# iKrishneel/fcn_object_detector

Measured on AMD Instinct MI355X. Metric: frames/sec forward 448x448 @1 GPU; train imgs/sec @1/2/4/8 GPUs, higher is better.
Workload: dtype f32; 1 GPU; configs[1]: single-GPU forward, DetectNet GoogLeNet conv stack + coverage/bbox heads (graph of models/deploy.prototxt), batch=1, 448x448, random-init weights; global_batch=1, parallelism=replicas x1, frames_in_flight=4

## Files before the change

### fcn_object_detector_amd/csrc/common.h

```cpp
#pragma once

#include <hip/hip_runtime.h>
#include <stdint.h>
#include <stdio.h>
#include <string.h>

#include "../../include/fcnhip.h"

namespace fcn {

char* err_buf();
int set_err(int code, const char* fmt, ...);

inline hipStream_t as_stream(fcn_stream_t s) { return reinterpret_cast<hipStream_t>(s); }

#define FCN_HIP(call)                                                                         \
    do {                                                                                      \
        hipError_t e__ = (call);                                                              \
        if (e__ != hipSuccess)                                                                \
            return ::fcn::set_err(-(int)e__, "%s failed: %s", #call, hipGetErrorString(e__)); \
    } while (0)

#define FCN_LAUNCH_CHECK(name)                                                                \
    do {                                                                                      \
        hipError_t e__ = hipGetLastError();                                                   \
        if (e__ != hipSuccess)                                                                \
            return ::fcn::set_err(-(int)e__, "launch %s failed: %s", name, hipGetErrorString(e__)); \
    } while (0)

#define FCN_REQUIRE(cond, code, ...)                         \
    do {                                                     \
        if (!(cond)) return ::fcn::set_err(code, __VA_ARGS__); \
    } while (0)

const float* zero_page_for_current_device(int* rc);

inline int cdiv(long long a, long long b) { return (int)((a + b - 1) / b); }

inline int stream_grid(long long work_items, int block) {
    long long g = (work_items + block - 1) / block;
    if (g < 1) g = 1;
    if (g > 65536) g = 8192;
    return (int)g;
}

}
```

### fcn_object_detector_amd/csrc/conv_fwd.hip

```cpp
#include <cstddef>
#include <algorithm>
#include <mutex>
#include <unordered_map>
#include <type_traits>

#include "common.h"
#include "conv_common.h"

using namespace fcn;

namespace fcn {

const float* zero_page_for_current_device(int* rc) {
    static std::mutex mu;
    static const float* pages[64] = {nullptr};
    int dev = 0;
    *rc = 0;
    if (hipGetDevice(&dev) != hipSuccess || dev < 0 || dev >= 64) {
        *rc = set_err(FCN_E_STATE, "conv: no current device");
        return nullptr;
    }
    std::lock_guard<std::mutex> lock(mu);
    if (!pages[dev]) {
        void* ptr = nullptr;
// ... 896 lines not shown
__global__ __launch_bounds__((Cfg<WTM, WTN, WAVES_M, WAVES_N, WAVES_K, BK, NBUF, PF>::NT)) void conv_fwd_group(const int nprob, const int te0, const int te1, const int te2,
                                                                                  const int te3, const int te4, const int te5, const int te6,
                                                                                  const int te7, const int pool_wgs, const int snake,
                                                                                  const std::conditional_t<TAIL, GroupArgsTail, GroupArgs> a_) {
    __shared__ __attribute__((aligned(16))) float smem[Cfg<WTM, WTN, WAVES_M, WAVES_N, WAVES_K, BK, NBUF, PF>::LDS_FLOATS + (TAIL ? kTailLdsFloats : 0)];
    const GroupArgs& a = group_of(a_);
    typedef unsigned u32x16 __attribute__((ext_vector_type(16)));
    typedef unsigned u32x8 __attribute__((ext_vector_type(8)));
    typedef const GroupArgs __attribute__((address_space(4))) * karg_ptr;
    static_assert(alignof(GroupArgsTail) == alignof(GroupArgs) && offsetof(GroupArgsTail, g) == 0, "the group leads its tail");
    constexpr size_t kArgsOffset = (11 * sizeof(int) + alignof(GroupArgs) - 1) / alignof(GroupArgs) * alignof(GroupArgs);
    karg_ptr ka = (karg_ptr)((const char __attribute__((address_space(4)))*)__builtin_amdgcn_kernarg_segment_ptr() + kArgsOffset);
    const int head[1 + kMaxGroup] = {nprob, te0, te1, te2, te3, te4, te5, te6, te7};
    static_assert(kMaxGroup == 8, "the tile prefix travels as eight scalar kernel arguments");
    const int pool_first = pool_wgs > 0 ? pool_wgs : 0;
    if ((int)blockIdx.x < pool_first || (pool_wgs < 0 && (int)blockIdx.x >= te7)) {
        const int w = pool_wgs < 0 ? (int)blockIdx.x - te7 : (int)blockIdx.x;
        if (w < a.pool[0].wg_end) pool_body<T, Cfg<WTM, WTN, WAVES_M, WAVES_N, WAVES_K, BK, NBUF, PF>::NT>(a.pool[0], w);
        else pool_body<T, Cfg<WTM, WTN, WAVES_M, WAVES_N, WAVES_K, BK, NBUF, PF>::NT>(a.pool[1], w - a.pool[0].wg_end);
        return;
    }
    int pos = blockIdx.x;
    if (snake > 0) {
        const int sh = snake & 255, rounds = snake >> 8;
        const int r = pos >> sh, j = pos & ((1 << sh) - 1);
        if (r > 0 && r < rounds - 1 && ((rounds - 1 - r) & 1)) pos = (r << sh) + ((1 << sh) - 1 - j);
    }
    int tile = pos - pool_first;
    if (snake == (int)0x80000000) {
        const int x = pos & 7, sl = pos >> 3, q = te7 >> 3, r = te7 & 7;
        tile = x * q + (x < r ? x : r) + sl;
    } else if (snake < 0) {
        tile += snake;
        tile += tile < 0 ? te7 : 0;
    }
    int pi = 0, begin = 0;
#pragma unroll
    for (int i = 0; i < kMaxGroup - 1; ++i) {
        const int end_i = head[1 + i];
        const bool past = i + 1 < nprob && tile >= end_i;
        pi += past ? 1 : 0;
        begin = past ? end_i : begin;
    }
    u32x16 ra, rb;
    u32x8 rc;
    pi = __builtin_amdgcn_readfirstlane(pi);
    begin = __builtin_amdgcn_readfirstlane(begin);
    const ConvP __attribute__((address_space(4)))* pbase = &ka->p[pi];
    asm volatile("s_load_dwordx16 %0, %3, 0x0\n\ts_load_dwordx16 %1, %3, 0x40\n\ts_load_dwordx8 %2, %3, 0x80\n\ts_waitcnt lgkmcnt(0)"
                 : "=&s"(ra), "=&s"(rb), "=&s"(rc)
                 : "s"(pbase)
                 : "memory");
    ConvP prob;
    __builtin_memcpy((char*)&prob, &ra, 64);
    __builtin_memcpy((char*)&prob + 64, &rb, 64);
    __builtin_memcpy((char*)&prob + 128, &rc, 32);
    if constexpr (TAIL) {
        tail_kptr tp = (tail_kptr)((const char __attribute__((address_space(4)))*)ka + offsetof(GroupArgsTail, tail));
        conv_body<T, WTM, WTN, WAVES_M, WAVES_N, WAVES_K, BK, NBUF, PF, true>(prob, tile - begin, smem, tp);
    } else {
        conv_body<T, WTM, WTN, WAVES_M, WAVES_N, WAVES_K, BK, NBUF, PF>(prob, tile - begin, smem);
    }
}

template <typename T, int WTM, int WTN, int WAVES_M, int WAVES_N, int WAVES_K, int BK, int NBUF, bool PF>
__global__ __launch_bounds__((Cfg<WTM, WTN, WAVES_M, WAVES_N, WAVES_K, BK, NBUF, PF>::NT)) void conv_fwd_one(ConvP p) {
    __shared__ __attribute__((aligned(16))) float smem[Cfg<WTM, WTN, WAVES_M, WAVES_N, WAVES_K, BK, NBUF, PF>::LDS_FLOATS];
    conv_body<T, WTM, WTN, WAVES_M, WAVES_N, WAVES_K, BK, NBUF, PF>(p, blockIdx.x, smem);
}

constexpr int kD7Th = 8, kD7Tw = 32;
constexpr int kD7Ph = 2 * kD7Th + 5, kD7Pw = 2 * kD7Tw + 6;
constexpr int kD7RowF = kD7Pw * 3;
constexpr int kD7PatchF = kD7Ph * kD7RowF;
constexpr int kD7WRowF = 22, kD7WPitchF = 7 * kD7WRowF;
constexpr int kD7WOff = (kD7PatchF + 3) / 4 * 4;
constexpr int kD7EpiPitch = 68;
constexpr int kD7StageF = kD7WOff + 64 * kD7WPitchF;
constexpr int kD7EpiF = 4 * 2 * 32 * kD7EpiPitch;
constexpr int kD7LdsBytes = (kD7StageF > kD7EpiF ? kD7StageF : kD7EpiF) * 4;
constexpr int kD7Threads = 256;
static_assert(kD7LdsBytes <= 80 * 1024, "first-layer kernel: two workgroups per CU");

__global__ __launch_bounds__(kD7Threads) void conv_first7_kernel(const ConvP p) {
#if defined(__HIP_DEVICE_COMPILE__)
    __shared__ __attribute__((aligned(16))) float smem[kD7LdsBytes / 4];
    const int tid = threadIdx.x, lane = tid & 63, wave = __builtin_amdgcn_readfirstlane(tid >> 6);
    FCN_STAMP(0);
    const int tiles_x = (p.OW + kD7Tw - 1) / kD7Tw, tiles_y = (p.OH + kD7Th - 1) / kD7Th;
    int t = blockIdx.x;
    const int tx = t % tiles_x;
    t /= tiles_x;
    const int ty = t % tiles_y, n = t / tiles_y;
    const int oy0 = ty * kD7Th, ox0 = tx * kD7Tw;
    const int iy0 = 2 * oy0 - 3, ix0 = 2 * ox0 - 3;
    const v4f zero4 = {0.f, 0.f, 0.f, 0.f};
    constexpr int PI = (kD7Ph * kD7Pw + kD7Threads - 1) / kD7Threads, WI = (64 * 49 + kD7Threads - 1) / kD7Threads;
    v4f px[PI], wv[WI];
    const float* xn = p.x + (size_t)n * p.H * p.W * 4;
#pragma unroll
    for (int i = 0; i < PI; ++i) {
        const int s = tid + kD7Threads * i;
        const int pr = s / kD7Pw, pc = s - pr * kD7Pw;
        const int iy = iy0 + pr, ix = ix0 + pc;
        const bool ok = s < kD7Ph * kD7Pw && (unsigned)iy < (unsigned)p.H && (unsigned)ix < (unsigned)p.W;
        px[i] = ok ? *reinterpret_cast<const v4f*>(xn + ((size_t)iy * p.W + ix) * 4) : zero4;
    }
#pragma unroll
    for (int i = 0; i < WI; ++i) {
        const int tp = tid + kD7Threads * i;
        wv[i] = tp < p.Cout * 49 ? *reinterpret_cast<const v4f*>(p.w + (size_t)tp * 4) : zero4;
    }
#pragma unroll
    for (int i = 0; i < PI; ++i) {
        const int s = tid + kD7Threads * i;
        if (s < kD7Ph * kD7Pw) {
            float* d = smem + s * 3;
            d[0] = px[i][0]; d[1] = px[i][1]; d[2] = px[i][2];
        }
    }
#pragma unroll
    for (int i = 0; i < WI; ++i) {
        const int tp = tid + kD7Threads * i;
        if (tp < 64 * 49) {
            const int co = tp / 49, rq = tp - co * 49;
            const int r = rq / 7, q = rq - r * 7;
            float* d = smem + kD7WOff + co * kD7WPitchF + r * kD7WRowF + q * 3;
            d[0] = wv[i][0]; d[1] = wv[i][1]; d[2] = wv[i][2];
        }
    }
    for (int i = tid; i < 64 * 7; i += kD7Threads) smem[kD7WOff + i * kD7WRowF + 21] = 0.f;
    const int c4 = (lane & 15) * 4;
    const v4f bias_v = (p.bias && c4 < p.Cout) ? *reinterpret_cast<const v4f*>(p.bias + c4) : zero4;
    FCN_STAMP(1);
    const int nl = lane & 31, h = lane >> 5;
    const float* a_base = smem + (4 * wave) * kD7RowF + 6 * nl + h;
    const float* b_base = smem + kD7WOff + nl * kD7WPitchF + h;
    typedef float v16f __attribute__((ext_vector_type(16)));
    v16f acc[2][2];
#pragma unroll
    for (int i = 0; i < 2; ++i)
#pragma unroll
        for (int j = 0; j < 2; ++j)
#pragma unroll
            for (int e = 0; e < 16; ++e) acc[i][j][e] = 0.f;
    __syncthreads();
    FCN_STAMP(2);
    auto frag = [&](const int step, float (&a)[2], float (&b)[2]) {
        const int r = step / 11, j = step - 11 * r;
#pragma unroll
        for (int mt = 0; mt < 2; ++mt) a[mt] = a_base[(2 * mt + r) * kD7RowF + 2 * j];
#pragma unroll
        for (int nt = 0; nt < 2; ++nt) b[nt] = b_base[nt * 32 * kD7WPitchF + r * kD7WRowF + 2 * j];
    };
    float fa[3][2], fb[3][2];
    frag(0, fa[0], fb[0]);
    frag(1, fa[1], fb[1]);
#pragma unroll
    for (int step = 0; step < 77; ++step) {
        if (step + 2 < 77) frag(step + 2, fa[(step + 2) % 3], fb[(step + 2) % 3]);
        __builtin_amdgcn_sched_barrier(0);
#pragma unroll
        for (int mt = 0; mt < 2; ++mt)
#pragma unroll
            for (int nt = 0; nt < 2; ++nt)
                acc[mt][nt] = __builtin_amdgcn_mfma_f32_32x32x2f32(fa[step % 3][mt], fb[step % 3][nt], acc[mt][nt], 0, 0, 0);
    }
    FCN_STAMP(3);
    __syncthreads();
    float* epi = smem + wave * (2 * 32 * kD7EpiPitch);
#pragma unroll
    for (int mt = 0; mt < 2; ++mt)
#pragma unroll
        for (int nt = 0; nt < 2; ++nt)
#pragma unroll
            for (int v = 0; v < 16; ++v) epi[(mt * 32 + (v & 3) + 8 * (v >> 2) + 4 * h) * kD7EpiPitch + nl + 32 * nt] = acc[mt][nt][v];
    asm volatile("s_waitcnt lgkmcnt(0)" ::: "memory");
    __builtin_amdgcn_sched_barrier(0);
    const bool do_relu = (p.flags & FCN_CONV_RELU) != 0;
#pragma unroll
    for (int mt = 0; mt < 2; ++mt) {
        const int oy = oy0 + 2 * wave + mt;
        float* yrow = p.y + ((size_t)(n * p.OH + oy) * p.OW + ox0) * p.y_cstride + p.y_coffset + c4;
#pragma unroll
        for (int i = 0; i < 8; ++i) {
            const int ox = (lane >> 4) + 4 * i;
            v4f v = *reinterpret_cast<const v4f*>(epi + (mt * 32 + ox) * kD7EpiPitch + c4) + bias_v;
            if (do_relu)
#pragma unroll
                for (int e = 0; e < 4; ++e) v[e] = fmaxf(v[e], 0.f);
            if (oy < p.OH && ox0 + ox < p.OW && c4 < p.Cout) *reinterpret_cast<v4f*>(yrow + (size_t)ox * p.y_cstride) = v;
        }
    }
#ifdef FCN_CONV_STAMPS
    FCN_STAMP(5);
    wait_vmcnt<0>();
    FCN_STAMP(6);
#endif
#endif
}

constexpr int kH7PatchSlots = (kD7Ph * kD7Pw + 63) / 64 * 64;
constexpr int kH7EpiOff = 2 * kH7PatchSlots * 16;
constexpr int kH7EpiPitch = 144;
constexpr int kH7LdsBytes = kH7EpiOff + 4 * 64 * kH7EpiPitch;
static_assert(kH7LdsBytes <= 160 * 1024, "half-float first-layer kernel: LDS image");

__global__ __launch_bounds__(kD7Threads) void conv_first7_f16_kernel(const ConvP p, const int ntiles) {
#if defined(__HIP_DEVICE_COMPILE__)
    __shared__ __attribute__((aligned(16))) char smem[kH7LdsBytes];
    const int tid = threadIdx.x, lane = tid & 63, wave = __builtin_amdgcn_readfirstlane(tid >> 6);
    const int tiles_x = (p.OW + kD7Tw - 1) / kD7Tw, tiles_y = (p.OH + kD7Th - 1) / kD7Th;
    const f16_t* xh = reinterpret_cast<const f16_t*>(p.x);
    const f16_t* wh = reinterpret_cast<const f16_t*>(p.w);
    f16_t* yh = reinterpret_cast<f16_t*>(p.y);
    const v4f zero4 = {0.f, 0.f, 0.f, 0.f};
    constexpr int PI = (kD7Ph * kD7Pw + kD7Threads - 1) / kD7Threads;
    auto fetch_patch = [&](const int tile, v4f (&px)[PI]) {
        int t = tile;
        const int tx = t % tiles_x;
        t /= tiles_x;
        const int ty = t % tiles_y, n = t / tiles_y;
        const int iy0 = 2 * ty * kD7Th - 3, ix0 = 2 * tx * kD7Tw - 3;
        const f16_t* xn = xh + (size_t)n * p.H * p.W * 8;
#pragma unroll
        for (int i = 0; i < PI; ++i) {
            const int s = tid + kD7Threads * i;
            const int pr = s / kD7Pw, pc = s - pr * kD7Pw;
            const int iy = iy0 + pr, ix = ix0 + pc;
            const bool ok = tile < ntiles && s < kD7Ph * kD7Pw && (unsigned)iy < (unsigned)p.H && (unsigned)ix < (unsigned)p.W;
            px[i] = ok ? *reinterpret_cast<const v4f*>(xn + ((size_t)iy * p.W + ix) * 8) : zero4;
        }
    };
    auto store_patch = [&](const int buf, const v4f (&px)[PI]) {
#pragma unroll
        for (int i = 0; i < PI; ++i) {
            const int s = tid + kD7Threads * i;
            if (s < kD7Ph * kD7Pw) *reinterpret_cast<v4f*>(smem + (buf * kH7PatchSlots + s) * 16) = px[i];
        }
    };
    const int nl = lane & 31, h = lane >> 5;
    v4f px[PI];
    int tile = blockIdx.x;
    fetch_patch(tile, px);
    v4f breg[28][2];
#pragma unroll
    for (int step = 0; step < 28; ++step)
#pragma unroll
        for (int nt = 0; nt < 2; ++nt) {
            const int r = step >> 2, q = (step & 3) + 4 * h, co = 2 * nl + nt;
            breg[step][nt] = (q < 7 && co < p.Cout) ? *reinterpret_cast<const v4f*>(wh + ((size_t)co * 49 + r * 7 + q) * 8) : zero4;
        }
    store_patch(0, px);
    const char* a_lane = smem + ((4 * wave) * kD7Pw + 2 * nl + 4 * h) * 16;
    const float bias0 = (p.bias && 2 * nl < p.Cout) ? p.bias[2 * nl] : 0.f;
    const float bias1 = (p.bias && 2 * nl + 1 < p.Cout) ? p.bias[2 * nl + 1] : 0.f;
    const bool do_relu = (p.flags & FCN_CONV_RELU) != 0;
    char* epi = smem + kH7EpiOff + wave * (64 * kH7EpiPitch);
    typedef float v16f __attribute__((ext_vector_type(16)));
    __syncthreads();
    int buf = 0;
    for (; tile < ntiles; tile += gridDim.x) {
        fetch_patch(tile + (int)gridDim.x, px);
        const char* a_base = a_lane + buf * kH7PatchSlots * 16;
        v16f acc[2][2];
#pragma unroll
        for (int i = 0; i < 2; ++i)
#pragma unroll
            for (int j = 0; j < 2; ++j)
#pragma unroll
                for (int e = 0; e < 16; ++e) acc[i][j][e] = 0.f;
        auto frag = [&](const int step, v4f (&a)[2]) {
            const int r = step >> 2, q = step & 3;
#pragma unroll
            for (int mt = 0; mt < 2; ++mt) a[mt] = *reinterpret_cast<const v4f*>(a_base + ((2 * mt + r) * kD7Pw + q) * 16);
        };
        v4f fa[3][2];
        frag(0, fa[0]);
        frag(1, fa[1]);
#pragma unroll
        for (int step = 0; step < 28; ++step) {
            if (step + 2 < 28) frag(step + 2, fa[(step + 2) % 3]);
// ... 186 lines not shown
                    acc[mt][nt] = __builtin_amdgcn_mfma_f32_32x32x16_f16(__builtin_bit_cast(v8h, fa[step % 3][mt]), __builtin_bit_cast(v8h, breg[step][nt]),
                                                                         acc[mt][nt], 0, 0, 0);
#endif
        }
        int tq = tile;
        const int tx = tq % tiles_x;
        tq /= tiles_x;
        const int ty = tq % tiles_y, n = tq / tiles_y;
        const bool border = ty == 0 || tx == 0 || 2 * (ty * kD7Th + kD7Th - 1) + 3 >= p.H || 2 * (tx * kD7Tw + kD7Tw - 1) + 3 >= p.W;
#pragma unroll
        for (int mt = 0; mt < 2; ++mt) {
            const int oy = ty * kD7Th + 2 * wave + mt;
            const int rlo = max(0, 3 - 2 * oy), rhi = min(7, p.H + 3 - 2 * oy);
#pragma unroll
            for (int v = 0; v < 16; ++v) {
                const int oxl = (v & 3) + 8 * (v >> 2) + 4 * h;
                float b0 = in0, b1 = in1;
                if (border) {
                    const int ox = tx * kD7Tw + oxl;
                    const int qlo = max(0, 3 - 2 * ox), qhi = min(7, p.W + 3 - 2 * ox);
                    if (rlo > 0 || rhi < 7 || qlo > 0 || qhi < 7) {
                        const int rh = max(rhi, rlo), qh = max(qhi, qlo);
                        const v2f a = *reinterpret_cast<const v2f*>(tab + (rh * 8 + qh) * 64 + 2 * nl), bq = *reinterpret_cast<const v2f*>(tab + (rlo * 8 + qh) * 64 + 2 * nl),
                                  cq = *reinterpret_cast<const v2f*>(tab + (rh * 8 + qlo) * 64 + 2 * nl), dq = *reinterpret_cast<const v2f*>(tab + (rlo * 8 + qlo) * 64 + 2 * nl);
                        b0 = bias0 + ((a[0] - bq[0]) - (cq[0] - dq[0]));
                        b1 = bias1 + ((a[1] - bq[1]) - (cq[1] - dq[1]));
                    }
                }
                typedef f16_t v2h __attribute__((ext_vector_type(2)));
                const v2f e = v2f{acc[mt][0][v], acc[mt][1][v]} + v2f{b0, b1};
                v2h pk = {(f16_t)e[0], (f16_t)e[1]};
                if (do_relu) pk = __builtin_elementwise_max(pk, v2h{(f16_t)0.f, (f16_t)0.f});
                *reinterpret_cast<v2h*>(epi + oxl * kX4EpiPitch + nl * 4) = pk;
            }
            asm volatile("s_waitcnt lgkmcnt(0)" ::: "memory");
            __builtin_amdgcn_sched_barrier(0);
            const int c8 = (lane & 7) * 8;
#pragma unroll
            for (int i = 0; i < 4; ++i) {
                const int ox = (lane >> 3) + 8 * i;
                const v4u val = *reinterpret_cast<const v4u*>(epi + ox * kX4EpiPitch + c8 * 2);
                const bool okp = oy < p.OH && tx * kD7Tw + ox < p.OW && c8 < p.Cout;
                int vo = okp ? (((n * p.OH + oy) * p.OW + tx * kD7Tw + ox) * p.y_cstride + p.y_coffset + c8) * 2 : OOB;
                asm volatile("" : "+v"(vo));
#ifdef FCN_X4_NOSTORE
                asm volatile("" ::"v"(val), "v"(vo));
#else
                __builtin_amdgcn_raw_buffer_store_b128(val, ry, vo, 0, 0);
#endif
            }
            asm volatile("s_waitcnt lgkmcnt(0)" ::: "memory");
            __builtin_amdgcn_sched_barrier(0);
        }
        asm volatile("s_waitcnt vmcnt(%0)" ::"n"(kX4PatchInstr / 4 + 8) : "memory");
        __builtin_amdgcn_s_barrier();
        asm volatile("" ::: "memory");
        buf = buf + 1 == kX4NBuf ? 0 : buf + 1;
    }
    asm volatile("s_waitcnt vmcnt(0)" ::: "memory");
#endif
}

bool first7_f16_ok(const ConvP& p) {
    return p.kh == 7 && p.kw == 7 && p.stride == 2 && p.pad == 3 && p.Cin == 8 && p.x_cstride == 8 && p.Cout > 32 && p.Cout <= 64 &&
           p.Cout % 8 == 0 && ((p.y_cstride | p.y_coffset) & 7) == 0 && ((uintptr_t)p.y & 15) == 0 &&
           (p.flags & ~(FCN_CONV_RELU | FCN_CONV_IMAGE_ONES)) == FCN_CONV_F16;
}

bool first7_ok(const ConvP& p) {
    return p.kh == 7 && p.kw == 7 && p.stride == 2 && p.pad == 3 && p.Cin == 4 && p.x_cstride == 4 && p.Cout > 32 && p.Cout <= 64 &&
           p.Cout % 4 == 0 && ((p.y_cstride | p.y_coffset) & 3) == 0 && ((uintptr_t)p.y & 15) == 0 && (!p.bias || ((uintptr_t)p.bias & 15) == 0) &&
           (p.flags & ~FCN_CONV_RELU) == 0;
}

constexpr int kDotPx = 4, kDotOut = 8, kDotMaxSlices = 4;
constexpr int kDotRedPx = 4;
constexpr int kDotRedPitch = 68;
struct DotSlice {
    const float* x;
    const float* w;
    const float* bias;
    float* y;
    float* y2;
    int K, x_cstride, y_cstride, y_coffset, y2_cstride, y2_coffset, nout, flags;
};
struct DotArgs {
    int M, nslices;
    DotSlice s[kDotMaxSlices];
};

__global__ __launch_bounds__(64 * kDotMaxSlices) void conv_dot1x1_kernel(const DotArgs a) {
    __shared__ __attribute__((aligned(16))) float red[kDotMaxSlices][kDotRedPx * kDotOut * kDotRedPitch];
    const int lane = threadIdx.x & 63, wave = __builtin_amdgcn_readfirstlane((int)threadIdx.x >> 6);
    if (wave >= a.nslices) return;
    DotSlice sl = a.s[0];
#pragma unroll
    for (int i = 1; i < kDotMaxSlices; ++i)
        if (wave == i) sl = a.s[i];
    const int m0 = blockIdx.x * kDotPx;
    const v4f zero4 = {0.f, 0.f, 0.f, 0.f};
    v4f acc[kDotPx][kDotOut];
#pragma unroll
    for (int p = 0; p < kDotPx; ++p)
#pragma unroll
        for (int o = 0; o < kDotOut; ++o) acc[p][o] = zero4;
    constexpr int U = 4;
    for (int k0 = lane * 4; k0 < sl.K; k0 += 256 * U) {
        v4f xa[U][kDotPx], wb[U][kDotOut];
#pragma unroll
        for (int u = 0; u < U; ++u) {
            const int k = k0 + 256 * u;
            const bool in = k < sl.K;
#pragma unroll
            for (int p = 0; p < kDotPx; ++p)
                xa[u][p] = in && m0 + p < a.M ? *reinterpret_cast<const v4f*>(sl.x + (size_t)(m0 + p) * sl.x_cstride + k) : zero4;
#pragma unroll
            for (int o = 0; o < kDotOut; ++o) wb[u][o] = in && o < sl.nout ? *reinterpret_cast<const v4f*>(sl.w + (size_t)o * sl.K + k) : zero4;
        }
#pragma unroll
        for (int u = 0; u < U; ++u)
#pragma unroll
            for (int p = 0; p < kDotPx; ++p)
#pragma unroll
                for (int o = 0; o < kDotOut; ++o) acc[p][o] += xa[u][p] * wb[u][o];
    }
    float* r = red[wave];
#pragma unroll
    for (int round = 0; round < kDotPx / kDotRedPx; ++round) {
#pragma unroll
        for (int p = 0; p < kDotRedPx; ++p)
#pragma unroll
            for (int o = 0; o < kDotOut; ++o) {
                const v4f t = acc[round * kDotRedPx + p][o];
                r[(p * kDotOut + o) * kDotRedPitch + lane] = (t[0] + t[1]) + (t[2] + t[3]);
            }
        asm volatile("s_waitcnt lgkmcnt(0)" ::: "memory");
        __builtin_amdgcn_sched_barrier(0);
        if (lane < kDotRedPx * kDotOut) {
            const int p = lane / kDotOut, o = lane % kDotOut;
            v4f q = *reinterpret_cast<const v4f*>(r + lane * kDotRedPitch);
#pragma unroll
            for (int j = 1; j < 16; ++j) q += *reinterpret_cast<const v4f*>(r + lane * kDotRedPitch + 4 * j);
            float v = (q[0] + q[1]) + (q[2] + q[3]);
            const int m = m0 + round * kDotRedPx + p;
            if (m < a.M && o < sl.nout) {
                if (sl.bias) v += sl.bias[o];
                if (sl.flags & FCN_CONV_RELU) v = fmaxf(v, 0.f);
                sl.y[(size_t)m * sl.y_cstride + sl.y_coffset + o] = v;
                if (sl.flags & FCN_CONV_SIGMOID2) sl.y2[(size_t)m * sl.y2_cstride + sl.y2_coffset + o] = 1.f / (1.f + expf(-v));
            }
        }
        asm volatile("s_waitcnt lgkmcnt(0)" ::: "memory");
        __builtin_amdgcn_sched_barrier(0);
    }
}

bool dot1x1_ok(const ConvP* ps, int n) {
    int slices = 0;
    for (int i = 0; i < n; ++i) {
        const ConvP& p = ps[i];
        if (p.kh != 1 || p.kw != 1 || p.stride != 1 || p.pad != 0 || (p.flags & ~(FCN_CONV_RELU | FCN_CONV_SIGMOID2)) != 0) return false;
        if (p.M != ps[0].M || p.Cin % 4 != 0) return false;
        slices += cdiv(p.Cout, kDotOut);
    }
    return slices <= kDotMaxSlices;
}


#define FCN_CONV_CONFIGS(X)            \
    X(0, 2, 2, 2, 2, 1, 32, 4, false)  \
    X(1, 2, 1, 2, 2, 1, 32, 4, false)  \
    X(2, 1, 1, 2, 2, 1, 32, 4, true)   \
    X(3, 1, 1, 4, 1, 1, 32, 4, true)   \
    X(4, 1, 1, 2, 1, 2, 64, 4, true)   \
    X(5, 1, 1, 1, 1, 4, 64, 4, true)   \
    X(6, 1, 1, 2, 2, 1, 64, 4, true)   \
    X(7, 1, 1, 1, 1, 4, 64, 6, true)   \
    X(8, 1, 1, 1, 1, 8, 64, 4, true)   \
    X(9, 1, 1, 2, 2, 2, 64, 4, true)   \
    X(10, 1, 1, 2, 2, 2, 32, 4, true)  \
    X(11, 2, 1, 2, 2, 2, 32, 4, true)  \
    X(12, 1, 1, 2, 1, 4, 64, 4, true)  \
    X(13, 2, 2, 2, 2, 2, 32, 3, false) \
    X(14, 1, 1, 2, 2, 1, 32, 3, false) \
    X(15, 2, 1, 2, 2, 1, 32, 3, false) \
    X(16, 1, 2, 2, 2, 1, 32, 3, false) \
    X(17, 1, 1, 1, 1, 4, 64, 3, false) \
    X(18, 1, 1, 1, 1, 4, 32, 4, true)  \
    X(19, 1, 1, 2, 1, 2, 32, 4, true)  \
    X(20, 1, 1, 2, 1, 2, 32, 3, false) \
    X(21, 1, 1, 1, 1, 4, 32, 3, false) \
    X(22, 1, 1, 4, 1, 1, 32, 3, false) \
    X(23, 1, 1, 1, 1, 4, 32, 16 + 4, true)  \
    X(24, 1, 1, 1, 1, 4, 64, 16 + 4, true)  \
    X(25, 1, 1, 2, 1, 2, 32, 16 + 4, true)  \
    X(26, 1, 1, 2, 2, 1, 32, 16 + 4, true)  \
    X(27, 1, 1, 1, 1, 4, 32, 16 + 6, true)  \
    X(28, 1, 1, 2, 2, 1, 64, 16 + 4, true)  \
    X(29, 2, 1, 2, 2, 1, 32, 16 + 4, true)

struct TileCfg { int bm, bn, bk; bool prefetch; };
constexpr int kCfgThreads[] = {
#define X(I, A, B, C_, D, E, F, G, H) Cfg<A, B, C_, D, E, F, G, H>::NT,
    FCN_CONV_CONFIGS(X)
#undef X
};
constexpr int kCfgLdsBytes[] = {
#define X(I, A, B, C_, D, E, F, G, H) Cfg<A, B, C_, D, E, F, G, H>::LDS_FLOATS * 4,
    FCN_CONV_CONFIGS(X)
#undef X
};
constexpr bool kCfgRoles[] = {
#define X(I, A, B, C_, D, E, F, G, H) Cfg<A, B, C_, D, E, F, G, H>::ROLES,
    FCN_CONV_CONFIGS(X)
#undef X
};
constexpr int kCfgWavesK[] = {
#define X(I, A, B, C_, D, E, F, G, H) E,
    FCN_CONV_CONFIGS(X)
#undef X
};
constexpr int kNumTileCfg = 30;
constexpr int kFirst7Cfg = kNumTileCfg;
constexpr int kDot1x1Cfg = kNumTileCfg + 1;
constexpr int kStreamCfg0 = kNumTileCfg + 2;
inline int num_cfgs() { return kStreamCfg0 + stream_num_cfgs(); }
inline bool is_stream_cfg(int cfg) { return cfg >= kStreamCfg0 && cfg < num_cfgs(); }
constexpr TileCfg kCfgs[kNumTileCfg] = {
#define X(I, A, B, C_, D, E, F, G, H) {Cfg<A, B, C_, D, E, F, G, H>::BM, Cfg<A, B, C_, D, E, F, G, H>::BN, F, H},
    FCN_CONV_CONFIGS(X)
#undef X
};
// ... 151 lines not shown
        const bool lean = lean_ok && xb < (1ll << 31) && wb < (1ll << 31) && taps <= 31 && (taps == 1 || 2ll * cpt * bke <= 3ll * ps[i].Cin);
        ps[i].lean_chunks = lean ? taps * cpt : 0;
        static const int light_min = getenv("FCN_CONV_LIGHT") ? atoi(getenv("FCN_CONV_LIGHT")) : 4;
        ps[i].kw_magic = (65536 + ps[i].kw - 1) / ps[i].kw;
        const bool big_tile = bm * bn > 32 * 32;
        if (lean && kCfgRoles[cfg] && light_min > 0 && (taps == 1 || cpt >= light_min || big_tile)) ps[i].kw_magic = -1;
    }
    return total;
}

int device_cus() {
    static int cached[64] = {};
    int dev = 0;
    if (hipGetDevice(&dev) != hipSuccess || dev < 0 || dev >= 64) return 256;
    if (cached[dev] == 0) {
        int v = 0;
        cached[dev] = (hipDeviceGetAttribute(&v, hipDeviceAttributeMultiprocessorCount, dev) == hipSuccess && v > 0) ? v : 256;
    }
    return cached[dev];
}

template <typename T>
void launch_one_cfg(int cfg, const ConvP& p, int total, hipStream_t st) {
    if (cfg == kFirst7Cfg) {
        if (p.flags & FCN_CONV_F16) {
            static const bool x4_ok = !(getenv("FCN_FIRST7_X4") && atoi(getenv("FCN_FIRST7_X4")) == 0);
            const bool small = (long long)p.N * p.H * p.W * 16 < (1ll << 31) &&
                               (((long long)p.N * p.OH * p.OW - 1) * p.y_cstride + p.y_coffset + p.Cout) * 2 < (1ll << 31);
            if ((p.flags & FCN_CONV_IMAGE_ONES) && x4_ok && small) {
                const int grid = total < 2 * device_cus() ? total : 2 * device_cus();
                hipLaunchKernelGGL(conv_first7_f16x4_kernel, dim3(grid), dim3(kD7Threads), 0, st, p, total);
                return;
            }
            const int grid = total < device_cus() ? total : device_cus();
            hipLaunchKernelGGL(conv_first7_f16_kernel, dim3(grid), dim3(kD7Threads), 0, st, p, total);
        } else {
            hipLaunchKernelGGL(conv_first7_kernel, dim3(total), dim3(kD7Threads), 0, st, p);
        }
        return;
    }
    switch (cfg) {
#define X(I, A, B, C_, D, E, F, G, H)                                                                                                 \
    case I:                                                                                                                           \
        hipLaunchKernelGGL((conv_fwd_one<T, A, B, C_, D, E, F, G, H>), dim3(total), dim3(Cfg<A, B, C_, D, E, F, G, H>::NT), 0, st, p); \
        break;
        FCN_CONV_CONFIGS(X)
#undef X
    }
}

template <typename T>
void launch_group_cfg(int cfg, const GroupArgs& ga, int pool_wgs, int snake, int total, hipStream_t st) {
    switch (cfg) {
#define X(I, A, B, C_, D, E, F, G, H)                                                                                                     \
    case I:                                                                                                                               \
        hipLaunchKernelGGL((conv_fwd_group<T, A, B, C_, D, E, F, G, H>), dim3(total), dim3(Cfg<A, B, C_, D, E, F, G, H>::NT), 0, st, ga.nprob,      \
                           ga.tile_end[0], ga.tile_end[1], ga.tile_end[2], ga.tile_end[3], ga.tile_end[4], ga.tile_end[5], ga.tile_end[6],          \
                           ga.tile_end[7], pool_wgs, snake, ga);                                                                                   \
        break;
        FCN_CONV_CONFIGS(X)
#undef X
    }
}

constexpr bool tail_cfg_ok(int cfg) { return cfg == 23 || cfg == 24 || cfg == 25 || cfg == 27; }
void launch_group_tail(int cfg, const GroupArgsTail& ga, int pool_wgs, int snake, int total, hipStream_t st) {
    const GroupArgs& g = ga.g;
    switch (cfg) {
#define XT(I, A, B, C_, D, E, F, G, H)                                                                                                         \
    case I:                                                                                                                                    \
        hipLaunchKernelGGL((conv_fwd_group<float, A, B, C_, D, E, F, G, H, true>), dim3(total), dim3(Cfg<A, B, C_, D, E, F, G, H>::NT), 0, st, g.nprob, \
                           g.tile_end[0], g.tile_end[1], g.tile_end[2], g.tile_end[3], g.tile_end[4], g.tile_end[5], g.tile_end[6],             \
                           g.tile_end[7], pool_wgs, snake, ga);                                                                                \
        break;
        XT(23, 1, 1, 1, 1, 4, 32, 16 + 4, true)
        XT(24, 1, 1, 1, 1, 4, 64, 16 + 4, true)
        XT(25, 1, 1, 2, 1, 2, 32, 16 + 4, true)
        XT(27, 1, 1, 1, 1, 4, 32, 16 + 6, true)
#undef XT
    }
}

struct HostTail { bool on; int finalize; int n; fcn_conv_desc heads[kTailMaxSlices]; float* scratch; unsigned* arrive; TailP t; };
struct HostGroup { int n; ConvP ps[16]; int npool; PoolP pools[kMaxPool]; HostTail tail; };
std::unordered_map<const void*, HostTail> g_tails;
std::mutex g_groups_mu;
std::unordered_map<const void*, HostGroup> g_groups;

}

extern "C" {

#ifdef FCN_CONV_STAMPS
int fcn_debug_conv_stamps(void* d_buf, int cap) {
    FCN_HIP(hipMemcpyToSymbol(HIP_SYMBOL(g_conv_stamps), &d_buf, sizeof(d_buf)));
    FCN_HIP(hipMemcpyToSymbol(HIP_SYMBOL(g_conv_stamps_cap), &cap, sizeof(cap)));
    return 0;
}
#endif

int fcn_conv2d_fwd_f32(const fcn_conv_desc* h_desc, fcn_stream_t s) {
    FCN_REQUIRE(h_desc, FCN_E_ARG, "fcn_conv2d_fwd_f32: null desc");
    int rc = validate(*h_desc);
    if (rc) return rc;
    const float* zp = zero_page_for_current_device(&rc);
    if (rc) return rc;
    ConvP p;
    fill(p, *h_desc, zp);
    const int cfg = choose_cfg(&p, 1);
    const int total = plan_tiles_cfg(cfg, &p, 1);
    FCN_REQUIRE(total > 0, FCN_E_UNSUPPORTED, "conv: too many tiles for the 32-bit tile decode");
    if (h_desc->flags & FCN_CONV_F16) launch_one_cfg<f16_t>(cfg, p, total, as_stream(s));
    else launch_one_cfg<float>(cfg, p, total, as_stream(s));
    FCN_LAUNCH_CHECK("conv_fwd_one");
    return 0;
}

size_t fcn_conv2d_group_workspace_bytes(int n) { return sizeof(ConvP) * (size_t)(n > 0 ? n : 0); }

int fcn_conv2d_num_configs(void) { return num_cfgs(); }

int fcn_conv2d_first_layer_config(void) { return kFirst7Cfg; }

int fcn_conv2d_config_lds_bytes(int cfg) {
    if (is_stream_cfg(cfg)) return stream_cfg_info(cfg - kStreamCfg0).lds_bytes;
    return cfg == kFirst7Cfg ? kD7LdsBytes :       cfg == kDot1x1Cfg ? kDotMaxSlices * kDotRedPx * kDotOut * kDotRedPitch * 4 : cfg >= 0 && cfg < kNumTileCfg ? kCfgLdsBytes[cfg] : -1;
}

int fcn_conv2d_config_waves_k(int cfg) { return cfg == kFirst7Cfg || cfg == kDot1x1Cfg || is_stream_cfg(cfg) ? 1 : cfg >= 0 && cfg < kNumTileCfg ? kCfgWavesK[cfg] : -1; }

int fcn_conv2d_group_prepare(const fcn_conv_desc* h_descs, int n, void* d_workspace, int cfg_request, fcn_conv_group* h_out) {
    return fcn_conv2d_group_prepare_fused(h_descs, n, nullptr, 0, d_workspace, cfg_request, h_out);
}

int fcn_conv2d_group_prepare_fused(const fcn_conv_desc* h_descs, int n, const fcn_pool_desc* h_pools, int npools, void* d_workspace,
                                   int cfg_request, fcn_conv_group* h_out) {
    FCN_REQUIRE(h_descs && h_out && d_workspace && n > 0 && n <= 16, FCN_E_ARG, "fcn_conv2d_group_prepare: need 1..16 problems, workspace, out");
    FCN_REQUIRE(cfg_request >= -1 && cfg_request < num_cfgs(), FCN_E_ARG, "fcn_conv2d_group_prepare: tile configuration %d out of range", cfg_request);
    FCN_REQUIRE(npools >= 0 && npools <= kMaxPool && (npools == 0 || (h_pools && n <= kMaxGroup)), FCN_E_ARG,
                "fcn_conv2d_group_prepare_fused: at most %d poolings, and only beside at most %d convolutions", kMaxPool, kMaxGroup);
    ConvP ps[16];
    int zrc = 0;
    const float* zp = zero_page_for_current_device(&zrc);
    if (zrc) return zrc;
    for (int i = 0; i < n; ++i) {
        int rc = validate(h_descs[i]);
        if (rc) return rc;
        FCN_REQUIRE(((h_descs[i].flags ^ h_descs[0].flags) & FCN_CONV_F16) == 0, FCN_E_ARG, "conv group: f32 and f16 problems cannot share a launch");
        fill(ps[i], h_descs[i], zp);
    }
    const int group_f16 = (h_descs[0].flags & FCN_CONV_F16) ? 1 : 0;
    PoolP pools[kMaxPool] = {};
    for (int i = 0; i < npools; ++i) {
        const fcn_pool_desc& d = h_pools[i];
        FCN_REQUIRE(d.x && d.y && d.N > 0 && d.H > 0 && d.W > 0 && d.C > 0 && d.k > 0 && d.stride > 0 && d.pad >= 0 && d.pad < d.k && d.OH > 0 &&
                        d.OW > 0, FCN_E_ARG, "fused maxpool: bad args");
        FCN_REQUIRE((d.OH - 1) * d.stride - d.pad < d.H && (d.OW - 1) * d.stride - d.pad < d.W, FCN_E_ARG,
                    "fused maxpool: last window starts outside the image");
        const int peps = group_f16 ? 8 : 4;
        FCN_REQUIRE((d.f16 ? 1 : 0) == group_f16, FCN_E_ARG, "fused maxpool: element type differs from the group's convolutions");
        FCN_REQUIRE(d.C % peps == 0 && d.x_cstride % peps == 0 && d.y_cstride % peps == 0 && d.y_coffset % peps == 0 && d.x_cstride >= d.C &&
                        d.y_coffset >= 0 && d.y_cstride >= d.y_coffset + d.C, FCN_E_ALIGN, "fused maxpool: channels / strides must be multiples of %d", peps);
        FCN_REQUIRE((((uintptr_t)d.x | (uintptr_t)d.y | (uintptr_t)d.idx) & 15) == 0, FCN_E_ALIGN, "fused maxpool: pointers must be 16-byte aligned");
        FCN_REQUIRE((long long)d.N * d.OH * d.OW * (d.C / peps) < (1ll << 30), FCN_E_UNSUPPORTED, "fused maxpool: too large");
        PoolP& q = pools[i];
        q.x = d.x; q.y = d.y; q.idx = d.idx;
        q.N = d.N; q.H = d.H; q.W = d.W; q.C = d.C; q.x_cstride = d.x_cstride; q.k = d.k; q.stride = d.stride; q.pad = d.pad;
        q.OH = d.OH; q.OW = d.OW; q.y_cstride = d.y_cstride; q.y_coffset = d.y_coffset;
        q.items = d.N * d.OH * d.OW * (d.C / peps);
        q.wg_end = 0;
    }
    HostTail tail = {};
    {
        std::lock_guard<std::mutex> lock(g_groups_mu);
        auto it = g_tails.find(d_workspace);
        if (it != g_tails.end()) tail = it->second;
    }
    if (tail.on) {
        const fcn_conv_desc& h0 = tail.heads[0];
        int contributors = 0;
        FCN_REQUIRE(n <= kMaxGroup && !group_f16, FCN_E_UNSUPPORTED, "conv tail: at most %d float32 problems in the launch", kMaxGroup);
        for (int i = 0; i < n; ++i) {
            const ConvP& q = ps[i];
            if ((const float*)q.y != h0.x) continue;
            FCN_REQUIRE(q.y_cstride == h0.x_cstride && q.M == h0.N * h0.H * h0.W && q.Cout % 32 == 0 && q.y_coffset % 32 == 0 && q.y_coffset + q.Cout <= h0.Cin &&
                            (q.flags & ~FCN_CONV_RELU) == 0 && ((uintptr_t)q.y & 15) == 0 && q.y_cstride % 4 == 0 && (!q.bias || ((uintptr_t)q.bias & 15) == 0),
                        FCN_E_UNSUPPORTED, "conv tail: a producer of the narrow problems' input must be a float32 bias + ReLU convolution over the same pixels "
                                           "that writes whole 32-channel groups of it");
            ps[i].flags |= FCN_CONV_TAILF;
            ++contributors;
        }
        FCN_REQUIRE(contributors > 0, FCN_E_ARG, "conv tail: no problem of this group writes the narrow problems' input");
    }
    int cfg = cfg_request >= 0 ? cfg_request : choose_cfg(ps, n);
    if (tail.on && cfg_request < 0 && !tail_cfg_ok(cfg)) cfg = 23;
    FCN_REQUIRE(!tail.on || tail_cfg_ok(cfg), FCN_E_UNSUPPORTED, "conv tail: configuration %d has no tail variant (23, 24, 25, 27 do)", cfg);
    const int total = plan_tiles_cfg(cfg, ps, n);
    if (tail.on && total > 0) {
        TailP& t = tail.t;
        t = TailP{};
        t.h.scratch = tail.scratch;
        t.h.arrive = tail.arrive;
        t.h.K = tail.heads[0].Cin;
        t.h.M = tail.heads[0].N * tail.heads[0].H * tail.heads[0].W;
        t.h.nslices = tail.n;
        int rows = 0;
        for (int i = 0; i < tail.n; ++i) {
            const fcn_conv_desc& h = tail.heads[i];
            TailSlice& sl = t.s[i];
            sl.bias = h.bias; sl.y = h.y; sl.y2 = h.y2;
            sl.o0 = rows; sl.nout = h.Cout; sl.y_cstride = h.y_cstride; sl.y_coffset = h.y_coffset; sl.y2_cstride = h.y2_cstride; sl.y2_coffset = h.y2_coffset;
            sl.flags = h.flags;
            for (int r = 0; r < h.Cout; r += 4) t.h.gw[(rows + r) / 4] = h.w + (size_t)r * h.Cin;
            rows += h.Cout;
        }
        for (int j = rows / 4; j < kTailRows / 4; ++j) t.h.gw[j] = t.h.gw[0];
        t.h.rows = rows;
        t.h.dbg = getenv("FCN_TAIL_DEBUG") ? atoi(getenv("FCN_TAIL_DEBUG")) : 0;
        t.h.need = 0;
        if (tail.finalize)
            for (int i = 0; i < n; ++i)
                if (ps[i].flags & FCN_CONV_TAILF) t.h.need += ps[i].tiles_n;
    }
    FCN_REQUIRE(!(is_stream_cfg(cfg) && (total == -2 || npools || n > kMaxGroup)), FCN_E_UNSUPPORTED,
                "conv group: configuration %d (persistent half-float streaming kernel) takes at most %d half problems with half outputs, "
                "bias + ReLU only, Cout / y_cstride / y_coffset multiples of 8, stride-1 1x1 / 3x3 / 5x5 filters with pad (k - 1) / 2 on images wide "
                "enough for its slab buffer (1x1 filters: the configurations with three slab buffers), and no poolings", cfg, kMaxGroup);
    FCN_REQUIRE(total != -2 && !((cfg == kFirst7Cfg || cfg == kDot1x1Cfg) && npools), FCN_E_UNSUPPORTED,
                "conv group: configuration %d is shape-specific (%d: one 7x7 / stride 2 / pad 3 problem on 4-channel pixels, 33..64 outputs; "
                "%d: 1x1 / stride 1 float32 problems over the same pixels, at most 32 output channels in slices of 8) and takes no poolings",
                cfg, kFirst7Cfg, kDot1x1Cfg);
    FCN_REQUIRE(total > 0, FCN_E_UNSUPPORTED, "conv group: too many tiles for the 32-bit tile decode");
    FCN_HIP(hipMemcpy(d_workspace, ps, sizeof(ConvP) * n, hipMemcpyHostToDevice));
    {
        std::lock_guard<std::mutex> lock(g_groups_mu);
        HostGroup& hg = g_groups[d_workspace];
        hg.n = n;
        for (int i = 0; i < n; ++i) hg.ps[i] = ps[i];
        hg.npool = npools;
        for (int i = 0; i < kMaxPool; ++i) hg.pools[i] = pools[i];
        hg.tail = tail;
    }
    h_out->d_probs = d_workspace;
    h_out->n = n;
    h_out->cfg = cfg;
    h_out->total_tiles = total;
    return 0;
}

int fcn_conv2d_group_release(void* d_workspace) {
    std::lock_guard<std::mutex> lock(g_groups_mu);
    g_groups.erase(d_workspace);
    g_tails.erase(d_workspace);
    return 0;
}

namespace {
int tail_check(const fcn_conv_tail* t) {
    FCN_REQUIRE(t && t->n >= 1 && t->n <= kTailMaxSlices, FCN_E_ARG, "conv tail: 1..%d narrow problems", kTailMaxSlices);
    int rows = 0;
    const fcn_conv_desc& h0 = t->heads[0];
    for (int i = 0; i < t->n; ++i) {
        const fcn_conv_desc& h = t->heads[i];
        int rc = validate(h);
        if (rc) return rc;
        FCN_REQUIRE(h.kh == 1 && h.kw == 1 && h.stride == 1 && h.pad == 0 && (h.flags & ~(FCN_CONV_RELU | FCN_CONV_SIGMOID2)) == 0, FCN_E_UNSUPPORTED,
                    "conv tail: the narrow problems are float32 1x1 / stride 1 convolutions (bias, ReLU, sigmoid second output)");
        FCN_REQUIRE(h.x == h0.x && h.x_cstride == h0.x_cstride && h.Cin == h0.Cin && h.N == h0.N && h.H == h0.H && h.W == h0.W, FCN_E_ARG,
                    "conv tail: the narrow problems read the same blob");
        FCN_REQUIRE(h.Cout % 4 == 0 && h.Cin % 32 == 0 && h.Cin <= 1024 && h.y_cstride % 4 == 0 && h.y_coffset % 4 == 0 && ((uintptr_t)h.y & 15) == 0 &&
                        (!h.bias || ((uintptr_t)h.bias & 15) == 0) && (!h.y2 || (((uintptr_t)h.y2 & 15) == 0 && h.y2_cstride % 4 == 0 && h.y2_coffset % 4 == 0)),
                    FCN_E_UNSUPPORTED, "conv tail: outputs in whole, 16-byte aligned groups of four channels; input channels in whole groups of 32, at most 1024");
        rows += h.Cout;
    }
    FCN_REQUIRE(rows <= kTailRows, FCN_E_UNSUPPORTED, "conv tail: at most %d output channels in all", kTailRows);
    return 0;
}
}

size_t fcn_conv2d_tail_scratch_bytes(const fcn_conv_tail* t) {
    if (tail_check(t)) return 0;
    size_t rows = 0;
    for (int i = 0; i < t->n; ++i) rows += (size_t)t->heads[i].Cout;
    return (size_t)(t->heads[0].Cin / 32) * (size_t)t->heads[0].N * t->heads[0].H * t->heads[0].W * rows * sizeof(float);
}

size_t fcn_conv2d_tail_arrive_bytes(const fcn_conv_tail* t) {
    if (tail_check(t)) return 0;
    return ((size_t)t->heads[0].N * t->heads[0].H * t->heads[0].W / 32 + 1) * sizeof(unsigned);
}

int fcn_conv2d_group_attach_tail(void* d_workspace, const fcn_conv_tail* t) {
    FCN_REQUIRE(d_workspace, FCN_E_ARG, "fcn_conv2d_group_attach_tail: null workspace");
    if (!t) {
        std::lock_guard<std::mutex> lock(g_groups_mu);
        g_tails.erase(d_workspace);
        return 0;
    }
    int rc = tail_check(t);
    if (rc) return rc;
    FCN_REQUIRE(t->scratch && t->arrive && ((uintptr_t)t->scratch & 15) == 0, FCN_E_ARG, "fcn_conv2d_group_attach_tail: scratch (16-byte aligned) and arrival words");
    HostTail ht = {};
    ht.on = true;
    ht.finalize = t->finalize ? 1 : 0;
    ht.n = t->n;
    for (int i = 0; i < t->n; ++i) ht.heads[i] = t->heads[i];
    ht.scratch = t->scratch;
    ht.arrive = reinterpret_cast<unsigned*>(t->arrive);
    std::lock_guard<std::mutex> lock(g_groups_mu);
    g_tails[d_workspace] = ht;
    return 0;
}

int fcn_conv2d_fwd_group_f32(const fcn_conv_group* g, fcn_stream_t s) {
    FCN_REQUIRE(g && g->d_probs && g->n > 0 && g->total_tiles > 0, FCN_E_ARG, "fcn_conv2d_fwd_group_f32: unprepared group");
    FCN_REQUIRE(g->cfg >= 0 && g->cfg < num_cfgs(), FCN_E_ARG, "fcn_conv2d_fwd_group_f32: bad cfg %d", g->cfg);
    HostGroup hg;
    {
        std::lock_guard<std::mutex> lock(g_groups_mu);
        auto it = g_groups.find(g->d_probs);
        FCN_REQUIRE(it != g_groups.end() && it->second.n == g->n, FCN_E_STATE, "fcn_conv2d_fwd_group_f32: group was not prepared by this library instance");
        hg = it->second;
    }
    if (g->cfg == kDot1x1Cfg) {
        FCN_REQUIRE(hg.npool == 0 && dot1x1_ok(hg.ps, hg.n), FCN_E_STATE, "fcn_conv2d_fwd_group_f32: group was not prepared for the lane-split 1x1 kernel");
        DotArgs da = {};
        da.M = hg.ps[0].M;
        for (int i = 0; i < hg.n; ++i)
            for (int n0 = 0; n0 < hg.ps[i].Cout; n0 += kDotOut) {
                const ConvP& q = hg.ps[i];
                DotSlice& d = da.s[da.nslices++];
                d.x = q.x; d.w = q.w + (size_t)n0 * q.K; d.bias = q.bias ? q.bias + n0 : nullptr; d.y = q.y; d.y2 = q.y2;
                d.K = q.K; d.x_cstride = q.x_cstride; d.y_cstride = q.y_cstride; d.y_coffset = q.y_coffset + n0;
                d.y2_cstride = q.y2_cstride; d.y2_coffset = q.y2_coffset + n0;
                d.nout = q.Cout - n0 < kDotOut ? q.Cout - n0 : kDotOut;
                d.flags = q.flags;
            }
        hipLaunchKernelGGL(conv_dot1x1_kernel, dim3(g->total_tiles), dim3(64 * kDotMaxSlices), 0, as_stream(s), da);
        FCN_LAUNCH_CHECK("conv_dot1x1");
        return 0;
    }
    if (g->cfg == kFirst7Cfg) {
        FCN_REQUIRE(hg.n == 1 && hg.npool == 0 && (first7_ok(hg.ps[0]) || first7_f16_ok(hg.ps[0])), FCN_E_STATE,
                    "fcn_conv2d_fwd_group_f32: group was not prepared for the first-layer kernel");
        launch_one_cfg<float>(kFirst7Cfg, hg.ps[0], g->total_tiles, as_stream(s));
        FCN_LAUNCH_CHECK("conv_first7");
        return 0;
    }
    if (is_stream_cfg(g->cfg)) {
        FCN_REQUIRE(hg.npool == 0 && hg.n <= kMaxGroup && (hg.ps[0].flags & FCN_CONV_F16), FCN_E_STATE, "fcn_conv2d_fwd_group_f32: group was not prepared for the streaming kernel");
        GroupArgs ga;
        ga.npool = 0;
        for (int i = 0; i < kMaxPool; ++i) ga.pool[i] = PoolP{};
        ga.nprob = hg.n;
        for (int i = 0; i < kMaxGroup; ++i) {
            const ConvP& src = hg.ps[i < hg.n ? i : hg.n - 1];
            ga.p[i] = src;
            ga.tile_end[i] = src.tile_end;
        }
        launch_stream(g->cfg - kStreamCfg0, ga, g->total_tiles, as_stream(s));
        FCN_LAUNCH_CHECK("conv_stream_f16");
        return 0;
    }
    for (int first = 0; first < hg.n; first += kMaxGroup) {
        GroupArgs ga;
        ga.npool = 0;
        for (int i = 0; i < kMaxPool; ++i) ga.pool[i] = PoolP{};
        ga.nprob = hg.n - first < kMaxGroup ? hg.n - first : kMaxGroup;
        const int base = first ? hg.ps[first - 1].tile_end : 0;
        for (int i = 0; i < kMaxGroup; ++i) {
            const ConvP& src = hg.ps[first + (i < ga.nprob ? i : ga.nprob - 1)];
            ga.p[i] = src;
            ga.tile_end[i] = src.tile_end - base;
        }
        int grid = ga.tile_end[ga.nprob - 1];
        int pool_wgs = 0;
        if (hg.npool > 0) {
            int end = 0;
            ga.npool = hg.npool;
            for (int i = 0; i < kMaxPool; ++i) {
                ga.pool[i] = hg.pools[i < hg.npool ? i : hg.npool - 1];
                const int per_wg = kCfgThreads[g->cfg] * (ga.pool[i].items <= kPoolSmallItems ? 1 : kPoolItemsPerThread);
                if (i < hg.npool) end += (ga.pool[i].items + per_wg - 1) / per_wg;
                ga.pool[i].wg_end = end;
            }
            grid += end;
            static const bool pool_last = getenv("FCN_POOL_LAST") && atoi(getenv("FCN_POOL_LAST")) == 1;
            pool_wgs = pool_last ? -end : end;
        }
        int snake = 0;
        {
            static const bool snake_ok = !(getenv("FCN_CONV_SNAKE") && atoi(getenv("FCN_CONV_SNAKE")) == 0);
            const int cus = device_cus();
            if (snake_ok && ga.nprob > 1 && (cus & (cus - 1)) == 0 && grid > 2 * cus && pool_wgs >= 0 && pool_wgs < cus) {
                int sh = 0;
                while ((1 << sh) < cus) ++sh;
                snake = ((grid + cus - 1) / cus) << 8 | sh;
            } else if (getenv("FCN_CONV_XCD") && atoi(getenv("FCN_CONV_XCD")) == 1 && pool_wgs == 0 && first == 0 && hg.n <= kMaxGroup) {
                snake = (int)0x80000000;
            } else if (snake_ok && ga.nprob > 1 && pool_wgs == 0 && grid > cus && grid <= 2 * cus) {
                snake = -(grid - cus);
            }
        }
        if (hg.tail.on) {
            FCN_REQUIRE(tail_cfg_ok(g->cfg) && hg.n <= kMaxGroup, FCN_E_STATE, "fcn_conv2d_fwd_group_f32: group was not prepared with its tail");
            GroupArgsTail gt;
            gt.g = ga;
            gt.tail = hg.tail.t;
            launch_group_tail(g->cfg, gt, pool_wgs, snake, grid, as_stream(s));
        } else if (hg.ps[0].flags & FCN_CONV_F16) launch_group_cfg<f16_t>(g->cfg, ga, pool_wgs, snake, grid, as_stream(s));
        else launch_group_cfg<float>(g->cfg, ga, pool_wgs, snake, grid, as_stream(s));
        FCN_LAUNCH_CHECK("conv_fwd_group");
    }
    return 0;
}

}
```

### fcn_object_detector_amd/csrc/runtime.hip

```cpp
#include <stdarg.h>

#include "common.h"

namespace fcn {

char* err_buf() {
    static thread_local char buf[512] = {0};
    return buf;
}

int set_err(int code, const char* fmt, ...) {
    va_list ap;
    va_start(ap, fmt);
    vsnprintf(err_buf(), 512, fmt, ap);
    va_end(ap);
    return code;
}

}

using namespace fcn;

extern "C" {

// ... 106 lines not shown
int fcn_event_destroy(fcn_event_t e) {
    if (e) FCN_HIP(hipEventDestroy((hipEvent_t)e));
    return 0;
}

int fcn_event_record(fcn_event_t e, fcn_stream_t s) {
    FCN_REQUIRE(e, FCN_E_ARG, "fcn_event_record: null");
    FCN_HIP(hipEventRecord((hipEvent_t)e, as_stream(s)));
    return 0;
}

int fcn_event_sync(fcn_event_t e) {
    FCN_REQUIRE(e, FCN_E_ARG, "fcn_event_sync: null");
    FCN_HIP(hipEventSynchronize((hipEvent_t)e));
    return 0;
}

int fcn_event_elapsed_ms(fcn_event_t start, fcn_event_t stop, float* h_ms) {
    FCN_REQUIRE(start && stop && h_ms, FCN_E_ARG, "fcn_event_elapsed_ms: null");
    FCN_HIP(hipEventElapsedTime(h_ms, (hipEvent_t)start, (hipEvent_t)stop));
    return 0;
}

int fcn_stream_wait_event(fcn_stream_t s, fcn_event_t e) {
    FCN_REQUIRE(e, FCN_E_ARG, "fcn_stream_wait_event: null event");
    FCN_HIP(hipStreamWaitEvent(as_stream(s), (hipEvent_t)e, 0));
    return 0;
}

int fcn_graph_begin(fcn_stream_t s) {
    FCN_REQUIRE(s, FCN_E_ARG, "fcn_graph_begin: capture needs an explicit stream");
    FCN_HIP(hipStreamBeginCapture(as_stream(s), hipStreamCaptureModeThreadLocal));
    return 0;
}

int fcn_graph_end(fcn_stream_t s, fcn_graph_t* g) {
    FCN_REQUIRE(s && g, FCN_E_ARG, "fcn_graph_end: null");
    hipGraph_t graph = nullptr;
    FCN_HIP(hipStreamEndCapture(as_stream(s), &graph));
    hipGraphExec_t exec = nullptr;
    hipError_t e = hipGraphInstantiate(&exec, graph, nullptr, nullptr, 0);
    (void)hipGraphDestroy(graph);
    if (e != hipSuccess) return set_err(-(int)e, "hipGraphInstantiate failed: %s", hipGetErrorString(e));
    *g = exec;
    return 0;
}

int fcn_graph_launch(fcn_graph_t g, fcn_stream_t s) {
    FCN_REQUIRE(g, FCN_E_ARG, "fcn_graph_launch: null");
    FCN_HIP(hipGraphLaunch((hipGraphExec_t)g, as_stream(s)));
    return 0;
}

int fcn_graph_destroy(fcn_graph_t g) {
    if (g) FCN_HIP(hipGraphExecDestroy((hipGraphExec_t)g));
    return 0;
}

int fcn_stream_create_replica(fcn_stream_t* s, int index) {
    FCN_REQUIRE(s, FCN_E_ARG, "fcn_stream_create_replica: null");
    if (index >= 0 && index < FCN_REPLICA_STREAMS) {
        int least = 0, greatest = 0;
        if (hipDeviceGetStreamPriorityRange(&least, &greatest) == hipSuccess && greatest < least) {
            hipStream_t st = nullptr;
            if (hipStreamCreateWithPriority(&st, hipStreamNonBlocking, greatest) == hipSuccess) {
                *s = st;
                return 0;
            }
        }
        (void)hipGetLastError();
    }
    return fcn_stream_create(s);
}

int fcn_stream_is_prioritized(fcn_stream_t s, int* h_yes) {
    FCN_REQUIRE(s && h_yes, FCN_E_ARG, "fcn_stream_is_prioritized: null");
    int least = 0, greatest = 0, prio = 0;
    FCN_HIP(hipDeviceGetStreamPriorityRange(&least, &greatest));
    FCN_HIP(hipStreamGetPriority(as_stream(s), &prio));
    *h_yes = (greatest < least && prio == greatest) ? 1 : 0;
    return 0;
}

}
```

### fcn_object_detector_amd/engine.py

```python
from __future__ import annotations

import ctypes as C
import os
import threading
from collections import namedtuple
from dataclasses import dataclass, field
from typing import Callable, Dict, List, Optional, Sequence, Tuple, Union

import numpy as np

from . import lib as L
from . import region as RG
from . import ssd as SSD
from . import storage as S
from . import tune as T
from .netspec import Layer, NetSpec, bn_global_stats, crop_window, interp_size, is_rectangular, kernel_stride_pad, layer_dilation, layer_geometry
from .storage import _r4, _ra, ip_pack_bank, ip_unpack_bank

F32 = np.float32


def graphs_enabled() -> bool:
    return os.environ.get("FCN_NO_GRAPH", "0") in ("", "0")

# ... 201 lines not shown
    def ptr(self) -> int:
        return self.buf.ptr + self.esize * self.coffset

    @property
    def contiguous(self) -> bool:
        return self.coffset == 0 and self.cstride == self.channels


class Op:

    def __init__(self, kind: str, name: str, run: Callable[[Optional[int]], None], flops: float = 0.0, bytes_: float = 0.0):
        self.kind = kind
        self.name = name
        self.run = run
        self.flops = flops
        self.bytes = bytes_


Range = Tuple[int, int, int]


@dataclass(eq=False)
class ConvTask:
    layer: Layer
    desc: L.ConvDesc
    flops: float
    bytes: float
    reads: List[Range]
    writes: List[Range]


@dataclass(eq=False)
class OpTask:
    layer: Layer
    ops: List[Op]
    reads: List[Range]
    writes: List[Range]
    pool_desc: Optional[L.PoolDesc] = None
    dconv: Optional[L.DConvDesc] = None
    rconv: Optional[L.RConvDesc] = None
    dwconv: Optional[L.DwConvDesc] = None


Task = Union[ConvTask, OpTask]


@dataclass(eq=False)
class BnChain:
    x: str
    y: str
    bn: Optional[Layer] = None
    scale: Optional[Layer] = None
    relu: Optional[Layer] = None
    mids: List[str] = field(default_factory=list)
    save: Optional["DeviceBuffer"] = None
    global_stats: bool = False


def ranges_hit(a: Sequence[Range], b: Sequence[Range]) -> bool:
    return any(x[0] == y[0] and x[1] < y[2] and y[1] < x[2] for x in a for y in b)


def task_waits(later: Task, earlier: Task) -> bool:
    return ranges_hit(later.reads, earlier.writes) or ranges_hit(later.writes, earlier.writes) or ranges_hit(later.writes, earlier.reads)


def task_levels(tasks: Sequence[Task], group_convs: bool = True) -> List[int]:
    levels: List[int] = []
    for i, ti in enumerate(tasks):
        levels.append(max([levels[j] + 1 for j in range(i) if task_waits(ti, tasks[j])], default=0) if group_convs else i)
    return levels


def task_floats(tasks: Sequence[Task], levels: Sequence[int], i: int) -> bool:
    return not any(levels[j] == levels[i] + 1 and task_waits(tj, tasks[i]) for j, tj in enumerate(tasks) if j != i)


class Engine:

    def __init__(self, spec: NetSpec, data_shapes: Optional[Dict[str, Tuple[int, ...]]] = None,
                 params: Optional[Dict[str, List[np.ndarray]]] = None, device: int = 0,
                 fuse: bool = True, group_convs: bool = True, autotune: bool = True, dtype: str = "f32",
                 tune_from: Optional["Engine"] = None, tune_max_lds_kb: Optional[int] = None,
                 share_params: Optional["Engine"] = None, score_outputs: bool = False, replica: Optional[int] = None):
        if dtype not in ("f32", "f16"):
            raise ValueError("dtype must be 'f32' or 'f16'")
        if share_params is not None and (dtype != "f32" or share_params.f16):
            raise NotImplementedError("share_params: only between float32 engines (a half-float engine packs its weights differently)")
        self._share_from = share_params
        self.shared_layers: set = set()
        self.score_outputs = bool(score_outputs)
        self.score_acc: Dict[str, DeviceBuffer] = {}
        self.graph_score: Optional[int] = None
        if dtype == "f16" and spec.phase != "TEST":
            raise NotImplementedError("the half-float path is inference only (BASELINE configs[4])")
        self.dtype, self.f16 = dtype, dtype == "f16"
        self.spec = spec
        self.device = device
        self.fuse = fuse
        self.group_convs = group_convs
        self.autotune = autotune
        L.call("fcn_init", device)
        sp = C.c_void_p()
        self.replica = replica if replica is not None else _take_replica_index()
        if self.replica is None:
            L.call("fcn_stream_create", C.byref(sp))
        else:
            L.call("fcn_stream_create_replica", C.byref(sp), int(self.replica))
        self.stream = int(sp.value)
        yes = C.c_int(0)
        L.call("fcn_stream_is_prioritized", self.stream, C.byref(yes))
        self.stream_prioritized = bool(yes.value)
        self.lock = threading.RLock()
        self.shapes = spec.infer(data_shapes)
        self.blobs: Dict[str, Blob] = {}
        self.params_host: Dict[str, List[np.ndarray]] = {}
        self.params_dev: Dict[str, List[DevView]] = {}
        self.ops: List[Op] = []
        self.graph_io: Optional[int] = None
        self.graph_core: Optional[int] = None
        self._staging: Dict[str, DeviceBuffer] = {}
        self._keep: List[object] = []
        self._conv_layer_meta: Dict[str, dict] = {}
        self._group_workspaces: List[DeviceBuffer] = []
        self.aux_dev: Dict[str, DeviceBuffer] = {}
        self._bn_chains: Dict[str, BnChain] = {}
        self._bn_ws_bytes = 0
        self._bn_ws: Optional[DeviceBuffer] = None
        self._lazy_blob_ops: Dict[str, List[Op]] = {}
        self.loss_blobs: Dict[str, float] = {}
        self.device_fed: set = set()
        self.dropout_seed = 0
        self.dropout_index_offset = 0
        self.inputs = spec.data_tops()
        self.outputs = [b for b in spec.output_blobs() if b in self.shapes and b not in spec.mask_blobs]
        max_lds = int(tune_max_lds_kb if tune_max_lds_kb is not None else os.environ.get("FCN_TUNE_MAX_LDS_KB", "160")) * 1024
        self.tuner = T.Tuner(self.stream, T.key_suffix(self.shapes.get(self.inputs[0], ()) if self.inputs else None, self.f16, max_lds),
                             spec.phase == "TEST", max_lds, tune_from._chosen_cfgs if tune_from is not None else None)
        self._plan_buffers()
        self._alloc_params(params)
        self._build_ops()
        self.tuner.release()

    @property
    def _chosen_cfgs(self) -> Dict[str, object]:
        return self.tuner.chosen

    def _plan_buffers(self) -> None:
        plan = S.plan_blobs(self.spec, self.shapes, self.inputs, self.outputs, self.f16, self.fuse, os.environ.get("FCN_F16_IMAGE", "1") != "0")
        self.producers, self.consumers = plan.producers, plan.consumers
        self.alias, self.shift, self.copy_concats, self.copy_slices = plan.alias, plan.shift, plan.copy_concats, plan.copy_slices
        self._half_inputs = plan.half_inputs
        self.permutes, self.gathers, self.detections = plan.permutes, plan.gathers, plan.detections
        self.pair_softmax, self.rpn_views = plan.pair_softmax, plan.rpn_views
        self.roi_counts: Dict[str, DeviceBuffer] = {}
        self._roi_count_host: Dict[str, "PinnedArray"] = {}
        self._roi_caps: Dict[str, int] = {}
        self._counts_valid = False
        bufs = {root: DeviceBuffer(nbytes) for root, nbytes in plan.root_bytes.items()}
        for name, v in plan.views.items():
            b = self.blobs[name] = Blob(name, v.shape)
            b.esize, b.rows, b.is_input = v.esize, v.rows, name in self.inputs
            b.buf, b.coffset, b.cstride = bufs[v.root], v.coffset, v.cstride
            b.upload_shift, b.lazy_shift = v.upload_shift, v.lazy_shift
        self._upload_priors()
        for d in self._half_inputs:
            b = self.blobs[d]
            ones = np.zeros((b.pixels, b.cstride), np.float16)
            ones[:, 3:5] = 1.0
            L.call("fcn_memcpy_h2d_async", b.buf.ptr, ones.ctypes.data, ones.nbytes, None)
            L.call("fcn_device_sync")

    def _upload_priors(self) -> None:
        self.prior_consts: Dict[str, np.ndarray] = {}
        for name, l in self.spec.prior_blobs.items():
            if l.type == "PriorBox":
                _, _, fh, fw = self.shapes[l.bottoms[0]]
                _, _, dh, dw = self.shapes[l.bottoms[1]]
                a = SSD.prior_boxes(SSD.priorbox_params(l), fh, fw, dh, dw)
            else:
                a = np.concatenate([self.prior_consts[b] for b in l.bottoms], axis=2)
            if a.shape != tuple(self.shapes[name]):
                raise RuntimeError("layer %s: %s prior constants for the blob %s" % (l.name, a.shape, self.shapes[name]))
            self.prior_consts[name] = a = np.ascontiguousarray(a, F32)
            b = self.blobs[name]
            if b.coffset or b.cstride != a.size:
                raise NotImplementedError("layer %s: the prior blob %s is a window of another buffer" % (l.name, name))
            L.call("fcn_memcpy_h2d_async", b.buf.ptr, a.ctypes.data, a.nbytes, None)
            L.call("fcn_device_sync")

    def _alloc_params(self, params: Optional[Dict[str, List[np.ndarray]]]) -> None:
        from .netspec import fill_params
        if params is None:
            params = fill_params(self.spec, seed=0)
        self.param_segs: Dict[Tuple[str, int], S.ParamSeg] = {}
        src = self._share_from
        if src is not None:
            self._shared_keep = [src.param_flat] + list(getattr(src, "_shared_keep", []))
            for l in self.spec.param_layers():
                if l.name not in src.params_dev:
                    continue
                mine, theirs = [tuple(x) for x in self.spec.param_shapes[l.name]], [tuple(x) for x in src.spec.param_shapes[l.name]]
                if mine != theirs:
                    raise ValueError("share_params: layer %s has blobs %s here and %s in the source net" % (l.name, mine, theirs))
                self.shared_layers.add(l.name)
                self.params_host[l.name] = src.params_host[l.name]
                self.params_dev[l.name] = [DevView(v.ptr, v.nbytes) for v in src.params_dev[l.name]]
                self.param_segs.update({(l.name, i): src.param_segs[(l.name, i)] for i in range(len(mine))})
        self.param_layout, self.param_count = S.param_layout(self.spec, self.blobs, self.f16, self.shared_layers)
        for l in self.spec.param_layers():
            if l.name in self.shared_layers:
                continue
            shapes = self.spec.param_shapes[l.name]
            blobs = params.get(l.name)
            if blobs is None:
                raise KeyError("no parameters for layer %s" % l.name)
            host = []
            for arr, shp in zip(blobs, shapes):
                a = np.ascontiguousarray(arr, dtype=F32)
                if a.shape != tuple(shp):
                    if a.size != int(np.prod(shp)):
                        raise ValueError("layer %s: parameter shape %s does not match %s" % (l.name, a.shape, shp))
                    a = a.reshape(shp)
                host.append(a.copy())
# ... 519 lines not shown

    def _dwconv_task(self, li: int, l: Layer, skip: set) -> OpTask:
        lib = L.load()
        g = self._dwgeom(l)
        xb, yb = self.blobs[l.bottoms[0]], self.blobs[l.tops[0]]
        eps = 16 // xb.esize
        if xb.coffset % eps or xb.cstride % eps:
            raise NotImplementedError("depthwise Convolution %s: input view is not 16-byte aligned" % l.name)
        if xb.esize == 4 and yb.esize != 4:
            raise NotImplementedError("f16 engine: depthwise Convolution %s reads the float32 blob %s and writes halves" % (l.name, l.bottoms[0]))
        relu = self._relu_after(li, l, skip)
        self._conv_layer_meta[l.name] = dict(relu=relu, sigmoid_top=None)
        pd = self.params_dev[l.name]
        flags = (L.CONV_RELU if relu else 0) | (L.CONV_OUT_F32 if xb.esize == 2 and yb.esize == 4 else 0)
        d = dwconv_desc(xb, yb, g, pd[0].ptr, pd[1].ptr if len(pd) > 1 else None, flags)
        fn = lib.fcn_dwconv2d_fwd_f16 if xb.esize == 2 else lib.fcn_dwconv2d_fwd_f32
        op = Op("dwconv", "%s [%dx%d]" % (l.name, g.kh, g.kw), lambda st: L.check(fn(C.byref(d), -1, st)), g.flops, g.bytes)
        return OpTask(l, [op], reads=[self._range(l.bottoms[0])], writes=[self._range(l.tops[0])], dwconv=d)

    def _rconv_task(self, li: int, l: Layer, skip: set) -> OpTask:
        kh, kw, sh, sw, ph, pw = layer_geometry(l)
        what = "%dx%d stride %dx%d pad %dx%d" % (kh, kw, sh, sw, ph, pw)
        if self.f16:
            raise NotImplementedError("f16 engine: rectangular Convolution %s (%s) has no half-float kernel" % (l.name, what))
        if self._conv_groups(l) > 1:
            raise NotImplementedError("rectangular Convolution %s (%s): group %d" % (l.name, what, self._conv_groups(l)))
        g = self._rgeom(l)
        xb, yb = self.blobs[l.bottoms[0]], self.blobs[l.tops[0]]
        if xb.coffset % 4 or xb.cstride % 4:
            raise NotImplementedError("rectangular Convolution %s: input view is not 16-byte aligned" % l.name)
        relu = self._relu_after(li, l, skip)
        self._conv_layer_meta[l.name] = dict(relu=relu, sigmoid_top=None)
        pd = self.params_dev[l.name]
        d = rconv_desc(xb, yb, g, pd[0].ptr, pd[1].ptr if len(pd) > 1 else None, L.CONV_RELU if relu else 0)
        return OpTask(l, [], reads=[self._range(l.bottoms[0])], writes=[self._range(l.tops[0])], rconv=d)

    def _emit_rconvs(self, items: List[OpTask]) -> None:
        lib = L.load()
        by_bottom: Dict[Range, List[OpTask]] = {}
        for it in items:
            by_bottom.setdefault(it.reads[0], []).append(it)
        for chunk in by_bottom.values():
            arr = (L.RConvDesc * len(chunk))(*[it.rconv for it in chunk])
            ws = DeviceBuffer(int(lib.fcn_rconv2d_workspace_bytes(arr, len(chunk))), zero=False)
            plan = L.RConvPlan()
            L.call("fcn_rconv2d_prepare", arr, len(chunk), ws.ptr, -1, C.byref(plan))
            self._keep.extend([arr, ws, plan])
            geoms = [self._rgeom(it.layer) for it in chunk]
            label = "%s [%s %dwg]" % ("+".join(it.layer.name for it in chunk), ",".join("%dx%d" % (g.kh, g.kw) for g in geoms), plan.total_tiles)
            self.ops.append(Op("rconv", label, lambda st, p=plan: L.check(lib.fcn_rconv2d_f32(C.byref(p), st)),
                               sum(g.flops for g in geoms), sum(g.bytes for g in geoms)))

    def _emit_group(self, chunk: List[ConvTask], fused: List[OpTask], tail: Optional[dict]) -> None:
        lib = L.load()
        name = "+".join(it.layer.name for it in chunk)
        flops = sum(it.flops for it in chunk)
        byts = sum(it.bytes for it in chunk)
        arr = (L.ConvDesc * len(chunk))(*[it.desc for it in chunk])
        ws = DeviceBuffer(int(lib.fcn_conv2d_group_workspace_bytes(len(chunk))), zero=False)
        self._group_workspaces.append(ws)
        grp = L.ConvGroup()
        parr = (L.PoolDesc * max(len(fused), 1))(*[pt.pool_desc for pt in fused])
        tune_key = name + ("{+%d pool}" % len(fused) if fused else "")
        tailed = tail is not None and any(id(it) in tail["producers"] for it in chunk)
        if tailed:
            fin = 1 if any(tail["producers"][id(it)] == tail["final_level"] for it in chunk if id(it) in tail["producers"]) else 0
            tail["desc"].finalize = fin
            L.call("fcn_conv2d_group_attach_tail", ws.ptr, C.byref(tail["desc"]))
            tune_key += "{+tail%d}" % fin
            if fin:
                flops += sum(ht.flops for ht in tail["heads"])
                byts += sum(4.0 * ht.desc.Cout * (ht.desc.N * ht.desc.OH * ht.desc.OW + ht.desc.Cin) for ht in tail["heads"])
        cfg = self.tuner.conv_cfg(tune_key, arr, len(chunk), ws, parr, len(fused)) if self.autotune else -1
        L.call("fcn_conv2d_group_prepare_fused", arr, len(chunk), parr, len(fused), ws.ptr, cfg, C.byref(grp))
        self._keep.extend([arr, parr, ws, grp])
        kind = "conv_group" if len(chunk) > 1 else "conv"
        label = "%s [cfg%d %dwg]" % (name, grp.cfg, grp.total_tiles)
        if fused:
            label = "%s {+%s}" % (label, "+".join(pt.layer.name for pt in fused))
            byts += sum(pt.ops[0].bytes for pt in fused)
        if tailed:
            label = "%s {%s %s}" % (label, "tail:" if tail["desc"].finalize else "partial sums of", "+".join(ht.layer.name for ht in tail["heads"]))
        self.ops.append(Op(kind, label, lambda st, g=grp: L.check(lib.fcn_conv2d_fwd_group_f32(C.byref(g), st)), flops, byts))

    def _emit_convs(self, items: List[ConvTask], pools: List[OpTask], tail: Optional[dict]) -> None:
        for base in range(0, len(items), 16):
            chunk = items[base:base + 16]
            fused = pools[:2] if base == 0 and len(chunk) <= 8 else []
            parts = [chunk]
            if self.f16 and self.autotune and not fused and len(chunk) > 1:
                parts = self.tuner.split_level(chunk)
            for part in parts:
                self._emit_group(part, fused, tail)
                fused = []
            if base == 0 and len(chunk) <= 8:
                del pools[:2]
        for pt in pools:
            self.ops.extend(pt.ops)
        pools.clear()

    def _emit_score_ops(self) -> None:
        lib = L.load()
        for nm in self.outputs:
            b = self.blobs[nm]
            if b.esize != 4 or b.lazy_shift:
                raise NotImplementedError("score_outputs: output blob %s is not a plain float32 blob" % nm)
            count = int(np.prod(b.shape)) if b.shape else 1
            acc = DeviceBuffer(max(4 * count, 16), zero=True)
            self.score_acc[nm] = acc
            if b.nchw is not None:
                n, c, h, w = b.nchw
                args = (acc.ptr, b.buf.ptr, n, h * w, c, b.cstride, b.coffset)
            else:
                args = (acc.ptr, b.ptr, 1, 1, count, count, 0)
            self.ops.append(Op("score", "score:" + nm, lambda st, a=args: L.check(lib.fcn_score_accumulate_f32(*a, st)), 0.0, 12.0 * count))

    def _plan_tail(self, tasks: List[Task], levels: List[int]) -> Optional[dict]:
        if self.f16 or self.spec.phase != "TEST" or not (self.fuse and self.group_convs) or os.environ.get("FCN_CONV_TAIL", "0") != "1":
            return None
        conv_idx = [i for i, t in enumerate(tasks) if isinstance(t, ConvTask)]
        if not conv_idx:
            return None
        lh = max(levels[i] for i in conv_idx)
        heads = [i for i in conv_idx if levels[i] == lh]
        if any(levels[i] >= lh for i, t in enumerate(tasks) if not isinstance(t, ConvTask)) or not 1 <= len(heads) <= 4:
            return None
        d0 = tasks[heads[0]].desc
        m = d0.N * d0.OH * d0.OW
        rows = 0
        for i in heads:
            d = tasks[i].desc
            if (d.kh, d.kw, d.stride, d.pad) != (1, 1, 1, 0) or d.x != d0.x or d.x_cstride != d0.x_cstride or d.Cin != d0.Cin or d.Cin % 32 or d.Cin > 1024 or d.Cout % 4 \
                    or (d.flags & ~(L.CONV_RELU | L.CONV_SIGMOID2)) or d.y_cstride % 4 or d.y_coffset % 4 or (d.y2 and (d.y2_cstride % 4 or d.y2_coffset % 4)):
                return None
            rows += d.Cout
        if rows > 24 or m > 4096:
            return None
        xr = tasks[heads[0]].reads
        producers: Dict[int, int] = {}
        covered = 0
        for i, t in enumerate(tasks):
            if i in heads or not ranges_hit(t.writes, xr):
                continue
            if not isinstance(t, ConvTask):
                return None
            d = t.desc
            if levels[i] not in (lh - 1, lh - 2) or d.y != d0.x or d.y_cstride != d0.x_cstride or d.N * d.OH * d.OW != m \
                    or d.Cout % 32 or d.y_coffset % 32 or d.y_coffset + d.Cout > d0.Cin or (d.flags & ~L.CONV_RELU) or d.y_cstride % 4:
                return None
            producers[id(t)] = levels[i]
            covered += d.Cout
        if covered != d0.Cin or not producers:
            return None
        for lv in set(producers.values()):
            if sum(1 for i in conv_idx if levels[i] == lv) > 8:
                return None
        lib = L.load()
        desc = L.ConvTail()
        desc.n = len(heads)
        for j, i in enumerate(heads):
            desc.heads[j] = tasks[i].desc
        sb, ab = int(lib.fcn_conv2d_tail_scratch_bytes(C.byref(desc))), int(lib.fcn_conv2d_tail_arrive_bytes(C.byref(desc)))
        if sb <= 0 or ab <= 0:
            return None
        scratch, arrive = DeviceBuffer(sb, zero=False), DeviceBuffer(ab, zero=True)
        desc.scratch, desc.arrive = scratch.ptr, arrive.ptr
# ... 361 lines not shown
        for bn in l.bottoms:
            xb = self.blobs[bn]
            out.append(self._copy_op(l.name + ":" + bn, xb, xb.coffset, yb, yb.coffset + off, xb.pixels, xb.channels))
            off += xb.channels
        return out

    def _fwd_eltwise(self, l: Layer, halves: List[str]) -> List[Op]:
        lib, out = L.load(), []
        p = l.sub("eltwise_param")
        opname = str(p.get("operation", "SUM"))
        op = {"PROD": L.ELT_PROD, "SUM": L.ELT_SUM, "MAX": L.ELT_MAX}[opname]
        coeff = [float(c) for c in p.getall("coeff")] or [1.0] * len(l.bottoms)
        yb = self.blobs[l.tops[0]]
        srcs = [self.blobs[b] for b in l.bottoms]
        if halves and len(halves) != len(l.bottoms) + 1:
            raise NotImplementedError("f16 engine: Eltwise %s mixes half and float32 blobs" % l.name)
        for b in srcs + [yb]:
            if not (b.coffset == 0 and b.cstride == yb.cstride):
                raise NotImplementedError("Eltwise on channel slices (layer %s)" % l.name)
        count = yb.pixels * yb.cstride
        fn = lib.fcn_eltwise_fwd_f16 if halves else lib.fcn_eltwise_fwd_f32
        a = srcs[0]
        for i, b in enumerate(srcs[1:], start=1):
            ca = coeff[0] if i == 1 else 1.0
            out.append(Op("eltwise", l.name, lambda st, a=a, b=b, ca=ca, cb=coeff[i]: L.check(fn(
                a.ptr, b.ptr, yb.ptr, count, op, ca, cb, st)), 0.0, 3.0 * yb.esize * count))
            a = yb
        return out

    def _fwd_inner_product(self, l: Layer, relu: bool) -> List[Op]:
        lib = L.load()
        xb, yb = self.blobs[l.bottoms[0]], self.blobs[l.tops[0]]
        m, c, h, w = xb.nchw
        n_out = yb.channels
        k = h * w * xb.cstride
        if m > L.IP_MAX_ROWS:
            raise NotImplementedError("InnerProduct %s: a batch of %d rows (the streaming kernels take at most %d)" % (l.name, m, L.IP_MAX_ROWS))
        if xb.esize == 4 and yb.esize != 4:
            raise NotImplementedError("f16 engine: InnerProduct %s reads float32 and writes halves" % l.name)
        devs = self.params_dev[l.name]
        bias = devs[1].ptr if len(devs) > 1 else None
        nbytes = int(lib.fcn_inner_product_fwd_workspace_bytes(m, k, n_out, xb.esize))
        ws = DeviceBuffer(nbytes, zero=False) if nbytes else None
        if ws is not None:
            self._keep.append(ws)
        wsp = ws.ptr if ws is not None else None
        flags = (L.CONV_RELU if relu else 0) | L.IP_WEIGHTS_NT
        if xb.esize == 2:
            fn, flags = lib.fcn_inner_product_fwd_f16, flags | (L.CONV_OUT_F32 if yb.esize == 4 else 0)
        else:
            fn = lib.fcn_inner_product_fwd_f32
        wptr = devs[0].ptr
        return [Op("inner_product", l.name, lambda st: L.check(fn(xb.buf.ptr, k, wptr, bias, yb.buf.ptr, yb.cstride, yb.coffset, m, k, n_out,
                                                                  flags, wsp, st)),
                   2.0 * m * c * h * w * n_out, float(xb.esize) * (n_out * k + m * k) + float(yb.esize) * m * n_out)]

    def _fwd_deconvolution(self, l: Layer, halves: List[str]) -> List[Op]:
        lib = L.load()
        g = self._geom(l)
        xb, yb = self.blobs[l.bottoms[0]], self.blobs[l.tops[0]]
        c, co, k = g.cin, g.cout, g.k
        wdev = self.params_dev[l.name][0].ptr
        bdev = self.params_dev[l.name][1].ptr if len(self.params_dev[l.name]) > 1 else None
        if self.param_segs[(l.name, 0)].kind == S.DECONV:
            if xb.coffset % 4 or xb.cstride % 4:
                raise NotImplementedError("Deconvolution %s: input view is not 16-byte aligned" % l.name)
            bank = DeviceBuffer(max(int(lib.fcn_tconv_bank_floats(c, co, k, k)), 4) * 4, zero=True)
            d = tconv_desc(xb, yb, g, bank.ptr, bdev)
            tws = DeviceBuffer(int(lib.fcn_tconv2d_workspace_bytes(C.byref(d), 1)), zero=False)
            plan = L.TConvPlan()
            L.call("fcn_tconv2d_prepare", C.byref(d), 1, tws.ptr, -1, C.byref(plan))
            self._keep.extend([bank, d, tws, plan])
            return [Op("tconv_pack", l.name, lambda st: L.check(lib.fcn_tconv_bank_pack_f32(wdev, bank.ptr, c, co, _r4(co), k, k, st)),
                       0.0, 8.0 * c * co * k * k),
                    Op("tconv", l.name, lambda st: L.check(lib.fcn_tconv2d_f32(C.byref(plan), st)),
                       2.0 * g.n * g.h * g.w * c * co * k * k, 4.0 * (xb.pixels * c + yb.pixels * co))]
        if halves and (xb.esize != 2 or xb.coffset % 8):
            raise NotImplementedError("f16 engine: Deconvolution %s from a float32 blob / an unaligned channel slice" % l.name)
        fn, out_f32 = (lib.fcn_deconv_depthwise_fwd_f16, (1 if yb.esize == 4 else 0,)) if halves else (lib.fcn_deconv_depthwise_fwd_f32, ())
        return [Op("deconv", l.name, lambda st: L.check(fn(
            xb.ptr, wdev, bdev, yb.buf.ptr, g.n, g.h, g.w, c, xb.cstride, k, g.s, g.pad, g.oh, g.ow, yb.cstride, yb.coffset, *out_f32, st)),
            2.0 * yb.pixels * c * (k / g.s) ** 2, float(xb.esize * xb.pixels + yb.esize * yb.pixels) * c)]

    def _stage(self, name: str) -> DeviceBuffer:
        st = self._staging.get(name)
        if st is None:
            b = self.blobs[name]
            st = DeviceBuffer(max(int(np.prod(b.shape)) if b.shape else 1, 1) * 4, zero=False)
            self._staging[name] = st
        return st

    def host_array(self, name: str) -> np.ndarray:
        b = self.blobs[name]
        if b.host is None:
            b.pinned = PinnedArray(b.shape)
            b.host = b.pinned.array
        return b.host

    def _upload_copy(self, name: str, stream: Optional[int]) -> None:
        b = self.blobs[name]
        host = self.host_array(name)
        dst = b.ptr if b.nchw is None else self._stage(name).ptr
        L.check(L.load().fcn_memcpy_h2d_async(dst, host.ctypes.data, host.nbytes, stream))

    def _upload_convert(self, name: str, stream: Optional[int]) -> None:
        b = self.blobs[name]
        if b.nchw is None:
            return
        lib = L.load()
        n, c, h, w = b.nchw
        st = self._stage(name)
        if b.esize == 2:
            L.check(lib.fcn_nchw_f32_to_nhwc_f16(st.ptr, b.buf.ptr, n, c, h, w, b.cstride, b.coffset, b.upload_shift, stream))
        else:
            L.check(lib.fcn_nchw_to_nhwc_f32(st.ptr, b.buf.ptr, n, c, h, w, b.cstride, b.coffset, b.upload_shift, stream))

    def _download_convert(self, name: str, stream: Optional[int]) -> None:
        b = self.blobs[name]
        if b.nchw is None:
            return
        lib = L.load()
        n, c, h, w = b.nchw
        st = self._stage(name)
        if b.esize == 2:
            L.check(lib.fcn_nhwc_f16_to_nchw_f32(b.buf.ptr, st.ptr, n, c, h, w, b.cstride, b.coffset, stream))
        else:
            L.check(lib.fcn_nhwc_to_nchw_f32(b.buf.ptr, st.ptr, n, c, h, w, b.cstride, b.coffset, stream))

    def _download_convert_all(self, stream: Optional[int]) -> None:
        multi = [nm for nm in self.outputs if self.blobs[nm].nchw is not None and self.blobs[nm].esize == 4]
        if 2 <= len(multi) <= 8:
            if not hasattr(self, "_multi_descs"):
                arr = (L.LayoutDesc * len(multi))()
                for d, nm in zip(arr, multi):
                    b = self.blobs[nm]
                    n, c, h, w = b.nchw
                    d.src, d.dst, d.N, d.C, d.H, d.W, d.src_cstride, d.src_coffset = b.buf.ptr, self._stage(nm).ptr, n, c, h, w, b.cstride, b.coffset
                self._multi_descs = arr
            L.check(L.load().fcn_nhwc_to_nchw_multi_f32(self._multi_descs, len(multi), stream))
        else:
            multi = []
        for nm in self.outputs:
            if nm not in multi:
                self._download_convert(nm, stream)

    def _download_copy(self, name: str, stream: Optional[int]) -> None:
        b = self.blobs[name]
        host = self.host_array(name)
        src = b.ptr if b.nchw is None else self._stage(name).ptr
        L.check(L.load().fcn_memcpy_d2h_async(host.ctypes.data, src, host.nbytes, stream))

    def _enqueue_upload(self, name: str, stream: Optional[int]) -> None:
        self._upload_copy(name, stream)
        self._upload_convert(name, stream)

    def _enqueue_download(self, name: str, stream: Optional[int]) -> None:
        self._download_convert(name, stream)
        self._download_copy(name, stream)

    def read_blob(self, name: str) -> np.ndarray:
        if name in self.spec.mask_blobs:
            return self._read_mask(name)
        if name in self.rpn_views:
            return np.ascontiguousarray(self.read_blob(self.rpn_views[name])).reshape(self.shapes[name])
        if name in self.permutes:
            return np.ascontiguousarray(self.read_blob(self.permutes[name]).transpose(0, 2, 3, 1))
        if name in self.spec.prior_blobs:
            return self.prior_consts[name]
        if name in self.detections:
            with self.lock:
                L.call("fcn_init", self.device)
                b = self.blobs[name]
                self.host_array(name)
                if not b.host_valid:
                    self._enqueue_download(name, self.stream)
                    L.call("fcn_stream_sync", self.stream)
                    b.host_valid = True
                return self._compose_detections(name)
        with self.lock:
            L.call("fcn_init", self.device)
            b = self.blobs[name]
            host = self.host_array(name)
            if not b.host_valid:
                for op in self._lazy_blob_ops.get(name, ()):
                    op.run(self.stream)
                self._enqueue_download(name, self.stream)
                L.call("fcn_stream_sync", self.stream)
                if b.lazy_shift:
                    host += F32(b.lazy_shift)
                b.host_valid = True
            return self._cut_rois(name, host)

    def _read_mask(self, name: str) -> np.ndarray:
        with self.lock:
            L.call("fcn_init", self.device)
            n, c, ph, pw = self.shapes[name]
            idx = self.aux_dev[self.spec.mask_blobs[name].name]
            host = np.empty((n, c, ph, pw), F32)
            tmp = DeviceBuffer(host.nbytes, zero=False)
            try:
                L.call("fcn_pool_mask_to_nchw_f32", idx.ptr, tmp.ptr, n, ph, pw, c, self.stream)
                L.call("fcn_memcpy_d2h_async", host.ctypes.data, tmp.ptr, host.nbytes, self.stream)
                L.call("fcn_stream_sync", self.stream)
            finally:
                tmp.free()
            return host

    LABEL_TOPS = ("coverage-label", "bbox-label", "size-block", "obj-block", "coverage-block")

    def set_targets(self, rects: Sequence[Sequence[Sequence[int]]], labels: Sequence[Sequence[int]], stride: int,
                    iou_thresh: float = 0.1, tops: Sequence[str] = LABEL_TOPS) -> None:
        fg = self.blobs[tops[0]]
        n, c, gy, gx = fg.shape
        if len(rects) != n or len(labels) != n:
            raise ValueError("need boxes for %d images" % n)
        offs = np.zeros(n + 1, np.int32)
        flat_r, flat_l = [], []
        for i, (rs, ls) in enumerate(zip(rects, labels)):
            for r, lab in zip(rs, ls):
                if not 0 <= int(lab) < c:
                    raise IndexError("label %d outside [0, %d)" % (lab, c))
                flat_r.append([int(v) for v in r])
                flat_l.append(int(lab))
            offs[i + 1] = len(flat_r)
        if not hasattr(self, "_tgt"):
            cap = max(64 * n, 256)
            self._tgt = dict(cap=cap, rects=DeviceBuffer(cap * 16, zero=True), labels=DeviceBuffer(cap * 4, zero=True),
                             offs=DeviceBuffer((n + 1) * 4, zero=True))
        if len(flat_r) > self._tgt["cap"]:
            raise ValueError("too many boxes in one batch (%d > %d)" % (len(flat_r), self._tgt["cap"]))
        self._tgt.update(h_rects=np.asarray(flat_r, np.int32).reshape(-1, 4), h_labels=np.asarray(flat_l, np.int32), h_offs=offs,
                         stride=int(stride), thresh=float(iou_thresh), tops=tuple(tops), pending=True)

    def _enqueue_targets(self) -> None:
        t, lib = self._tgt, L.load()
        if t["h_rects"].size:
            L.check(lib.fcn_memcpy_h2d_async(t["rects"].ptr, t["h_rects"].ctypes.data, t["h_rects"].nbytes, self.stream))
            L.check(lib.fcn_memcpy_h2d_async(t["labels"].ptr, t["h_labels"].ctypes.data, t["h_labels"].nbytes, self.stream))
        L.check(lib.fcn_memcpy_h2d_async(t["offs"].ptr, t["h_offs"].ctypes.data, t["h_offs"].nbytes, self.stream))
        fg, bb, sz, ob, cv = (self.blobs[nm] for nm in t["tops"])
        n, c, gy, gx = fg.shape
        for b in (bb, sz, ob, cv):
            if b.coffset or b.cstride != bb.cstride:
                raise NotImplementedError("label blobs must be plain buffers of one geometry")
        L.check(lib.fcn_gen_targets_nhwc(t["rects"].ptr, t["labels"].ptr, t["offs"].ptr, n, c, gy, gx, t["stride"], t["thresh"],
                                         fg.ptr, fg.cstride, bb.ptr, sz.ptr, ob.ptr, cv.ptr, bb.cstride, self.stream))


    def score_begin(self, io: bool = False) -> None:
        if not self.score_outputs:
            raise RuntimeError("engine was not built with score_outputs=True")
        with self.lock:
            L.call("fcn_init", self.device)
            for nm in self.inputs:
                if nm not in self.device_fed:
                    self.host_array(nm)
                    if self.blobs[nm].nchw is not None:
                        self._stage(nm)
            if graphs_enabled():
                if io and self.graph_io is None:
                    for nm in self.outputs:
                        self.host_array(nm)
                    self.graph_io = self._capture(with_io=True)
                elif not io and self.graph_score is None:
                    self.graph_score = self._capture(with_io=True, download=False)
            for acc in self.score_acc.values():
                L.call("fcn_memset_async", acc.ptr, 0, acc.nbytes, self.stream)
            self.score_forwards = 0

    def forward_score(self, uploaded_event=None) -> None:
        with self.lock:
            for nm in self.inputs:
                if nm not in self.device_fed:
                    self._upload_copy(nm, self.stream)
            if uploaded_event is not None:
                L.call("fcn_event_record", uploaded_event, self.stream)
            if getattr(self, "_tgt", None) is not None and self._tgt.get("pending"):
                self._enqueue_targets()
            if self.graph_score is not None:
                L.call("fcn_graph_launch", self.graph_score, self.stream)
            else:
                for nm in self.inputs:
                    if nm not in self.device_fed:
                        self._upload_convert(nm, self.stream)
                self.run_ops(self.stream)
            for b in self.blobs.values():
                b.host_valid = False
            self.score_forwards += 1

    def score_read(self) -> Dict[str, np.ndarray]:
        with self.lock:
            out = {nm: np.empty(self.blobs[nm].shape, F32) for nm in self.outputs}
            for nm, a in out.items():
                L.call("fcn_memcpy_d2h_async", a.ctypes.data, self.score_acc[nm].ptr, a.nbytes, self.stream)
            L.call("fcn_stream_sync", self.stream)
            return out

    def run_ops(self, stream: Optional[int]) -> None:
        for op in self.ops:
            op.run(stream)

    def _capture(self, with_io: bool, download: bool = True) -> int:
        if with_io:
            for nm in list(self.inputs) + list(self.outputs):
                self.host_array(nm)
                if self.blobs[nm].nchw is not None:
                    self._stage(nm)
        if not getattr(self, "_warm", False):
            self.run_ops(self.stream)
            L.call("fcn_stream_sync", self.stream)
            self._warm = True
        if with_io and not getattr(self, "_warm_io", False):
            for nm in self.inputs:
                if nm not in self.device_fed:
                    self._enqueue_upload(nm, self.stream)
            self._download_convert_all(self.stream)
            for nm in self.outputs:
                self._download_copy(nm, self.stream)
            L.call("fcn_stream_sync", self.stream)
            self._warm_io = True
        L.call("fcn_graph_begin", self.stream)
        try:
            if with_io:
                for nm in self.inputs:
                    if nm not in self.device_fed:
                        self._upload_convert(nm, self.stream)
            self.run_ops(self.stream)
            if with_io and download:
                self._download_convert_all(self.stream)
        finally:
            g = C.c_void_p()
            L.call("fcn_graph_end", self.stream, C.byref(g))
        return int(g.value)

    def _launch_io(self) -> None:
        if self.graph_io is None:
            self.graph_io = self._capture(with_io=True)
        for nm in self.inputs:
            if nm not in self.device_fed:
                self._upload_copy(nm, self.stream)
        L.call("fcn_graph_launch", self.graph_io, self.stream)
        for nm in self.outputs:
            self._download_copy(nm, self.stream)
        self._download_counts(self.stream)

    def forward(self, use_graph: bool = True) -> Dict[str, np.ndarray]:
        use_graph = use_graph and graphs_enabled()
        with self.lock:
            L.call("fcn_init", self.device)
            for nm in self.inputs:
                self.host_array(nm)
            for nm in self.outputs:
                self.host_array(nm)
            if use_graph:
                self._launch_io()
            else:
                for nm in self.inputs:
                    if nm not in self.device_fed:
                        self._enqueue_upload(nm, self.stream)
                self.run_ops(self.stream)
                for nm in self.outputs:
                    self._enqueue_download(nm, self.stream)
                self._download_counts(self.stream)
            L.call("fcn_stream_sync", self.stream)
            for b in self.blobs.values():
                b.host_valid = False
            self._ran = self._counts_valid = True
            out = {}
            for nm in self.outputs:
                b = self.blobs[nm]
                if b.lazy_shift:
                    b.host += F32(b.lazy_shift)
                b.host_valid = True
                out[nm] = self._cut_rois(nm, b.host) if nm not in self.detections else self._compose_detections(nm)
            for nm in self.inputs:
                self.blobs[nm].host_valid = nm not in self.device_fed
            return out

    def forward_begin(self) -> None:
        with self.lock:
            L.call("fcn_init", self.device)
            for nm in list(self.inputs) + list(self.outputs):
                self.host_array(nm)
            if graphs_enabled():
                self._launch_io()
            else:
                for nm in self.inputs:
                    if nm not in self.device_fed:
                        self._enqueue_upload(nm, self.stream)
                self.run_ops(self.stream)
                for nm in self.outputs:
                    self._enqueue_download(nm, self.stream)
                self._download_counts(self.stream)

    def forward_end(self) -> Dict[str, np.ndarray]:
        with self.lock:
            L.call("fcn_stream_sync", self.stream)
            for b in self.blobs.values():
                b.host_valid = False
            self._ran = self._counts_valid = True
            out = {}
            for nm in self.outputs:
                b = self.blobs[nm]
                if b.lazy_shift:
                    b.host += F32(b.lazy_shift)
                b.host_valid = True
                out[nm] = self._cut_rois(nm, b.host) if nm not in self.detections else self._compose_detections(nm)
            for nm in self.inputs:
                self.blobs[nm].host_valid = nm not in self.device_fed
            return out

    def upload_inputs(self) -> None:
        with self.lock:
            for nm in self.inputs:
                self._enqueue_upload(nm, self.stream)
            L.call("fcn_stream_sync", self.stream)

    def forward_enqueue(self) -> None:
        with self.lock:
            if graphs_enabled():
                if self.graph_core is None:
                    self.graph_core = self._capture(with_io=False)
                L.call("fcn_graph_launch", self.graph_core, self.stream)
            else:
                self.run_ops(self.stream)
            for b in self.blobs.values():
                if not b.is_input:
                    b.host_valid = False
            self._ran, self._counts_valid = True, False

    def forward_resident(self, iters: int = 1, use_graph: bool = True) -> float:
        use_graph = use_graph and graphs_enabled()
        with self.lock:
            L.call("fcn_init", self.device)
            if use_graph and self.graph_core is None:
                self.graph_core = self._capture(with_io=False)
            e0, e1 = C.c_void_p(), C.c_void_p()
            L.call("fcn_event_create", C.byref(e0))
            L.call("fcn_event_create", C.byref(e1))
            L.call("fcn_event_record", e0, self.stream)
            for _ in range(iters):
                if use_graph:
                    L.call("fcn_graph_launch", self.graph_core, self.stream)
                else:
                    self.run_ops(self.stream)
            L.call("fcn_event_record", e1, self.stream)
            L.call("fcn_event_sync", e1)
            ms = C.c_float()
            L.call("fcn_event_elapsed_ms", e0, e1, C.byref(ms))
            L.call("fcn_event_destroy", e0)
            L.call("fcn_event_destroy", e1)
            for b in self.blobs.values():
                if not b.is_input:
                    b.host_valid = False
            self._counts_valid = False
            return float(ms.value)

    def time_ops(self, reps: int = 20, ops: Optional[Sequence["Op"]] = None) -> List[Tuple[str, str, float, float, float]]:
        out = []
        with self.lock:
            e0, e1 = C.c_void_p(), C.c_void_p()
            L.call("fcn_event_create", C.byref(e0))
            L.call("fcn_event_create", C.byref(e1))
            for op in (self.ops if ops is None else ops):
                op.run(self.stream)
                L.call("fcn_event_record", e0, self.stream)
                for _ in range(reps):
                    op.run(self.stream)
                L.call("fcn_event_record", e1, self.stream)
                L.call("fcn_event_sync", e1)
                ms = C.c_float()
                L.call("fcn_event_elapsed_ms", e0, e1, C.byref(ms))
                out.append((op.kind, op.name, ms.value / reps, op.flops, op.bytes))
            L.call("fcn_event_destroy", e0)
            L.call("fcn_event_destroy", e1)
        return out

    def time_ops_in_sequence(self, reps: int = 10) -> List[Tuple[str, str, float, float, float]]:
        out = []
        with self.lock:
            e0, e1 = C.c_void_p(), C.c_void_p()
            L.call("fcn_event_create", C.byref(e0))
            L.call("fcn_event_create", C.byref(e1))
            ms = C.c_float()
            empty = []
            for _ in range(10):
                self.ops[0].run(self.stream)
                L.call("fcn_event_record", e0, self.stream)
                L.call("fcn_event_record", e1, self.stream)
                L.call("fcn_event_sync", e1)
                L.call("fcn_event_elapsed_ms", e0, e1, C.byref(ms))
                empty.append(ms.value)
            floor = float(np.median(empty))
            for i, op in enumerate(self.ops):
                acc = []
                for _ in range(reps):
                    for prev in self.ops[:i]:
                        prev.run(self.stream)
                    L.call("fcn_event_record", e0, self.stream)
                    op.run(self.stream)
                    L.call("fcn_event_record", e1, self.stream)
                    L.call("fcn_event_sync", e1)
                    L.call("fcn_event_elapsed_ms", e0, e1, C.byref(ms))
                    acc.append(ms.value)
                out.append((op.kind, op.name, float(np.median(acc)), op.flops, op.bytes))
            L.call("fcn_event_destroy", e0)
            L.call("fcn_event_destroy", e1)
        self.event_pair_floor_ms = floor
        return out

    def close(self) -> None:
        with self.lock:
            lib = L.load()
            for g in (self.graph_io, self.graph_core, self.graph_score):
                if g:
                    lib.fcn_graph_destroy(g)
            self.graph_io = self.graph_core = self.graph_score = None
            if self.stream:
                lib.fcn_stream_sync(self.stream)
                lib.fcn_stream_destroy(self.stream)
                self.stream = 0
            for ws in getattr(self, "_group_workspaces", []):
                if ws.ptr:
                    lib.fcn_conv2d_group_release(ws.ptr)
                    ws.free()
            self._group_workspaces = []
            self.ops = []
            self.tuner.release()

    def __del__(self):
        try:
            self.close()
        except Exception:
            pass


class ForwardPipeline:

    def __init__(self, make_spec: Callable[[], NetSpec], params: Optional[Dict[str, List[np.ndarray]]] = None, device: int = 0, depth: int = 4,
                 max_lds_kb: Optional[int] = 36, **engine_kw):
        if depth < 1:
            raise ValueError("depth must be at least 1")
        self.engines: List[Engine] = []
        if os.environ.get("FCN_PIPE_LDS_KB"):
            max_lds_kb = int(os.environ["FCN_PIPE_LDS_KB"]) or None
        if max_lds_kb is not None:
            engine_kw.setdefault("tune_max_lds_kb", max_lds_kb)
        for i in range(depth):
            self.engines.append(Engine(make_spec(), params=params, device=device, tune_from=self.engines[0] if i else None, replica=i,
                                       **engine_kw))
        self._pending: List[Engine] = []
        self._next = 0

    @property
    def depth(self) -> int:
        return len(self.engines)

    def submit(self, inputs: Dict[str, np.ndarray]) -> None:
        if len(self._pending) >= len(self.engines):
            raise RuntimeError("ForwardPipeline: %d frames already in flight, collect() one first" % len(self._pending))
        eng = self.engines[self._next]
        self._next = (self._next + 1) % len(self.engines)
        for nm, arr in inputs.items():
            eng.host_array(nm)[...] = arr
        eng.forward_begin()
        self._pending.append(eng)

    def collect(self) -> Dict[str, np.ndarray]:
        if not self._pending:
            raise RuntimeError("ForwardPipeline: nothing in flight")
        eng = self._pending.pop(0)
        return {k: v.copy() for k, v in eng.forward_end().items()}

    def map(self, frames: Sequence[Dict[str, np.ndarray]]) -> List[Dict[str, np.ndarray]]:
        out: List[Dict[str, np.ndarray]] = []
        for f in frames:
            if len(self._pending) == len(self.engines):
                out.append(self.collect())
            self.submit(f)
        while self._pending:
            out.append(self.collect())
        return out

    def calibrate(self, depths: Sequence[int] = (3, 4), iters: int = 60) -> int:
        best, best_t = None, 1e30
        for d in depths:
            if 1 <= d <= len(self.engines):
                self.run_resident(iters, depth=d)
                t = self.run_resident(iters, depth=d)
                if t < best_t:
                    best, best_t = d, t
        self.active = best or len(self.engines)
        return self.active

    def run_resident(self, iters: int, depth: Optional[int] = None) -> float:
        import time
        lib = L.load()
        engines = self.engines[:depth or getattr(self, "active", None) or len(self.engines)]
        return self._run_resident(engines, iters, lib, time)

    def run_io(self, iters: int, depth: Optional[int] = None) -> float:
        import time
        engines = self.engines[:depth or getattr(self, "active", None) or len(self.engines)]
        pending: List[Engine] = []
        t0 = time.perf_counter()
        for i in range(iters):
            e = engines[i % len(engines)]
            if len(pending) == len(engines):
                pending.pop(0).forward_end()
            e.forward_begin()
            pending.append(e)
        while pending:
            pending.pop(0).forward_end()
        return time.perf_counter() - t0

    def warm_io(self, depth: Optional[int] = None) -> None:
        for e in self.engines[:depth or getattr(self, "active", None) or len(self.engines)]:
            e.forward_begin()
            e.forward_end()

    def _run_resident(self, engines, iters, lib, time) -> float:
        for e in engines:
            if e.graph_core is None:
                e.forward_resident(1)
            L.call("fcn_stream_sync", e.stream)
        no_graph = not graphs_enabled()
        t0 = time.perf_counter()
        for i in range(iters):
            e = engines[i % len(engines)]
            if no_graph:
                e.run_ops(e.stream)
            else:
                L.check(lib.fcn_graph_launch(e.graph_core, e.stream))
        for e in engines:
            L.call("fcn_stream_sync", e.stream)
        return time.perf_counter() - t0

    def close(self) -> None:
        for e in self.engines:
            e.close()
```

### fcn_object_detector_amd/lib.py

```python
from __future__ import annotations

import ctypes as C
import os
import threading
from typing import Optional

_HERE = os.path.dirname(os.path.abspath(__file__))
LIB_PATH = os.environ.get("FCN_LIB_PATH") or os.path.join(_HERE, "libfcnhip.so")


class FcnLibraryError(RuntimeError):
    pass


class FcnError(RuntimeError):
    def __init__(self, code: int, msg: str):
        super().__init__("libfcnhip error %d: %s" % (code, msg))
        self.code = code


class ConvDesc(C.Structure):
    _fields_ = [
        ("x", C.c_void_p), ("w", C.c_void_p), ("bias", C.c_void_p), ("y", C.c_void_p), ("y2", C.c_void_p),
        ("N", C.c_int32), ("H", C.c_int32), ("W", C.c_int32), ("Cin", C.c_int32), ("x_cstride", C.c_int32),
# ... 106 lines not shown
                ("gray_alpha", C.c_float), ("gray_keep", C.c_float)]


GAUSS_MAX_RADIUS = 15
REPLICA_STREAMS = 4


class FlipSeg(C.Structure):
    _fields_ = [("w_offset", C.c_uint64), ("wt_offset", C.c_uint64), ("Cout", C.c_int32), ("kh", C.c_int32), ("kw", C.c_int32),
                ("Cin", C.c_int32), ("Cin4", C.c_int32), ("Cout4", C.c_int32)]


class DetectParams(C.Structure):
    _fields_ = [
        ("num_classes", C.c_int32), ("gy", C.c_int32), ("gx", C.c_int32), ("cell_w", C.c_int32), ("cell_h", C.c_int32),
        ("cvg_cstride", C.c_int32), ("cvg_coffset", C.c_int32), ("box_cstride", C.c_int32), ("box_coffset", C.c_int32),
        ("prob_thresh", C.c_float), ("group_thresh", C.c_int32), ("eps", C.c_double), ("min_height", C.c_int32),
        ("round_mode", C.c_int32), ("max_out", C.c_int32),
    ]


class SsdHead(C.Structure):
    _fields_ = [("src", C.c_void_p)] + [(k, C.c_int32) for k in ("pixels", "C", "cstride", "coffset", "dst_col", "reserved")]


class DetOutParams(C.Structure):
    _fields_ = [(k, C.c_int32) for k in ("N", "P", "num_classes", "background", "code_type", "variance_encoded", "top_k", "keep_top_k")] + [
        ("conf_threshold", C.c_float), ("nms_threshold", C.c_float)] + [(k, C.c_int32) for k in ("loc_rstride", "conf_rstride", "capacity", "reserved")]


class ProposalParams(C.Structure):
    _fields_ = [(k, C.c_int32) for k in ("H", "W", "A", "feat_stride", "pre_nms_topn", "post_nms_topn")] + [
        ("min_size", C.c_float), ("nms_thresh", C.c_float)] + [(k, C.c_int32) for k in (
            "score_cstride", "score_coffset", "delta_cstride", "delta_coffset", "rois_cstride", "rois_coffset", "top_score_cstride",
            "top_score_coffset")] + [("anchors", C.c_float * 128)]


PROPOSAL_MAX_ANCHORS = 32
PROPOSAL_MAX_CANDIDATES = 65536
PROPOSAL_MAX_PRE_NMS = 6144
SSD_MAX_HEADS = 16
DETOUT_MAX_TOPK = 1024
CODE_CORNER, CODE_CENTER_SIZE = 1, 2
CONV_RELU, CONV_SIGMOID2, CONV_ACCUM, CONV_OUT_F32, CONV_F16, CONV_OUT_F16, CONV_MASK = 1, 2, 4, 8, 16, 32, 64
IP_MAX_ROWS = 32
IP_WEIGHTS_NT = 256
CONV_IMAGE_ONES = 128
ELT_PROD, ELT_SUM, ELT_MAX = 0, 1, 2
SOLVER_KINDS = {"SGD": 0, "NESTEROV": 1, "ADAGRAD": 2, "RMSPROP": 3, "ADADELTA": 4, "ADAM": 5}
REG_L2, REG_L1 = 0, 1
RECT_ROUND_NEAREST_EVEN, RECT_ROUND_TRUNCATE = 0, 1

_vp, _i, _f, _d, _sz = C.c_void_p, C.c_int, C.c_float, C.c_double, C.c_size_t

PROTOTYPES = {
    "fcn_abi_version": (_i, []),
    "fcn_last_error_string": (C.c_char_p, []),
    "fcn_device_count": (_i, [C.POINTER(_i)]),
    "fcn_init": (_i, [_i]),
    "fcn_device_name": (_i, [C.c_char_p, _i]),
    "fcn_device_sync": (_i, []),
    "fcn_malloc": (_i, [C.POINTER(_vp), _sz]),
    "fcn_free": (_i, [_vp]),
    "fcn_host_malloc": (_i, [C.POINTER(_vp), _sz]),
    "fcn_host_free": (_i, [_vp]),
    "fcn_memset_async": (_i, [_vp, _i, _sz, _vp]),
    "fcn_memcpy_h2d_async": (_i, [_vp, _vp, _sz, _vp]),
    "fcn_memcpy_d2h_async": (_i, [_vp, _vp, _sz, _vp]),
    "fcn_memcpy_d2d_async": (_i, [_vp, _vp, _sz, _vp]),
    "fcn_stream_create": (_i, [C.POINTER(_vp)]),
    "fcn_stream_destroy": (_i, [_vp]),
    "fcn_stream_sync": (_i, [_vp]),
    "fcn_event_create": (_i, [C.POINTER(_vp)]),
    "fcn_event_destroy": (_i, [_vp]),
    "fcn_event_record": (_i, [_vp, _vp]),
    "fcn_event_sync": (_i, [_vp]),
    "fcn_event_elapsed_ms": (_i, [_vp, _vp, C.POINTER(_f)]),
    "fcn_graph_begin": (_i, [_vp]),
    "fcn_graph_end": (_i, [_vp, C.POINTER(_vp)]),
    "fcn_graph_launch": (_i, [_vp, _vp]),
    "fcn_graph_destroy": (_i, [_vp]),
    "fcn_stream_create_replica": (_i, [C.POINTER(_vp), _i]),
    "fcn_stream_is_prioritized": (_i, [_vp, C.POINTER(_i)]),
    "fcn_nchw_to_nhwc_f32": (_i, [_vp, _vp, _i, _i, _i, _i, _i, _i, _f, _vp]),
    "fcn_nhwc_to_nchw_f32": (_i, [_vp, _vp, _i, _i, _i, _i, _i, _i, _vp]),
    "fcn_nhwc_to_nchw_multi_f32": (_i, [C.POINTER(LayoutDesc), _i, _vp]),
    "fcn_conv2d_fwd_f32": (_i, [C.POINTER(ConvDesc), _vp]),
    "fcn_conv2d_group_workspace_bytes": (_sz, [_i]),
    "fcn_conv2d_num_configs": (_i, []),
    "fcn_conv2d_first_layer_config": (_i, []),
    "fcn_conv2d_config_lds_bytes": (_i, [_i]),
    "fcn_conv2d_config_waves_k": (_i, [_i]),
    "fcn_conv2d_group_prepare": (_i, [C.POINTER(ConvDesc), _i, _vp, _i, C.POINTER(ConvGroup)]),
    "fcn_conv2d_group_prepare_fused": (_i, [C.POINTER(ConvDesc), _i, C.POINTER(PoolDesc), _i, _vp, _i, C.POINTER(ConvGroup)]),
    "fcn_conv2d_fwd_group_f32": (_i, [C.POINTER(ConvGroup), _vp]),
    "fcn_conv2d_group_release": (_i, [_vp]),
    "fcn_conv2d_tail_scratch_bytes": (C.c_size_t, [C.POINTER(ConvTail)]),
    "fcn_conv2d_tail_arrive_bytes": (C.c_size_t, [C.POINTER(ConvTail)]),
    "fcn_conv2d_group_attach_tail": (_i, [_vp, C.POINTER(ConvTail)]),
    "fcn_maxpool_fwd_f32": (_i, [_vp, _vp, _vp] + [_i] * 12 + [_vp]),
    "fcn_avepool_fwd_f32": (_i, [_vp, _vp] + [_i] * 12 + [_vp]),
    "fcn_lrn_fwd_f32": (_i, [_vp, _vp, _vp, _i, _i, _i, _i, _i, _f, _f, _f, _vp]),
    "fcn_maxpool_lrn5_fwd_f32": (_i, [_vp, _vp] + [_i] * 12 + [_f, _f, _f, _vp]),
    "fcn_maxpool_lrn5_fwd_f16": (_i, [_vp, _vp] + [_i] * 12 + [_f, _f, _f, _vp]),
    "fcn_maxpool_lrn5_conv1x1_fwd_f32": (_i, [_vp] + [_i] * 10 + [_f, _f, _f, _vp, _vp, _i, _i, _vp, _i, _i, _vp]),
    "fcn_maxpool_lrn5_conv1x1_fwd_f16": (_i, [_vp] + [_i] * 10 + [_f, _f, _f, _vp, _vp, _i, _i, _vp, _i, _i, _vp]),
    "fcn_relu_fwd_f32": (_i, [_vp, _vp, _sz, _f, _vp]),
    "fcn_sigmoid_fwd_f32": (_i, [_vp, _vp, _sz, _vp]),
    "fcn_power_fwd_f32": (_i, [_vp, _vp, _sz, _f, _f, _f, _vp]),
    "fcn_eltwise_fwd_f32": (_i, [_vp, _vp, _vp, _sz, _i, _f, _f, _vp]),
    "fcn_copy_channels_f32": (_i, [_vp, _vp, _i, _i, _i, _i, _i, _i, _vp]),
    "fcn_deconv_depthwise_fwd_f32": (_i, [_vp, _vp, _vp, _vp] + [_i] * 12 + [_vp]),
    "fcn_preprocess_bgr8": (_i, [_vp, _i, _i, _vp, _i, _i, _i, _f, _vp, _vp]),
    "fcn_detect_workspace_bytes": (_sz, [C.POINTER(DetectParams), _i]),
    "fcn_detect_decode_group": (_i, [_vp, _vp, _i, _sz, _sz, C.POINTER(DetectParams), _vp, _vp, _vp, _vp, _vp]),
    "fcn_score_masks_workspace_bytes": (_sz, [_i, _i, _i, _i]),
    "fcn_score_masks": (_i, [_vp, _i, _i, _i, _i, _i, _i, _vp, _f, _vp, _i, _i, _vp, _vp, _vp]),
    "fcn_gen_targets": (_i, [_vp, _vp, _vp, _i, _i, _i, _i, _i, _d, _vp, _vp, _vp, _vp, _vp, _vp]),
    "fcn_gen_targets_nhwc": (_i, [_vp, _vp, _vp, _i, _i, _i, _i, _i, _d, _vp, _i, _vp, _vp, _vp, _vp, _i, _vp]),
    "fcn_conv2d_wgrad_workspace_floats": (_sz, [C.POINTER(ConvDesc), C.POINTER(_i)]),
    "fcn_conv2d_wgrad_f32": (_i, [C.POINTER(ConvDesc), _vp, _vp, _vp, _vp]),
    "fcn_conv2d_wgrad_group_workspace_floats": (_sz, [C.POINTER(ConvDesc), _i]),
    "fcn_conv2d_wgrad_group_f32": (_i, [C.POINTER(ConvDesc), _vp, _vp, _i, _vp, _vp]),
    "fcn_conv2d_wgrad_num_configs": (_i, []),
    "fcn_conv2d_wgrad_split_config": (_i, []),
    "fcn_conv2d_wgrad_workspace_floats_cfg": (_sz, [C.POINTER(ConvDesc), _i, C.POINTER(_i)]),
    "fcn_conv2d_wgrad_cfg_f32": (_i, [C.POINTER(ConvDesc), _vp, _vp, _vp, _i, _vp]),
    "fcn_conv2d_wgrad_group_workspace_floats_cfg": (_sz, [C.POINTER(ConvDesc), _i, _i]),
    "fcn_conv2d_wgrad_group_cfg_f32": (_i, [C.POINTER(ConvDesc), _vp, _vp, _i, _vp, _i, _vp]),
    "fcn_conv_weights_flip_f32": (_i, [_vp, _vp, _i, _i, _i, _i, _i, _i, _vp]),
    "fcn_nchw_f32_to_nhwc_f16": (_i, [_vp, _vp, _i, _i, _i, _i, _i, _i, _f, _vp]),
    "fcn_nhwc_f16_to_nchw_f32": (_i, [_vp, _vp, _i, _i, _i, _i, _i, _i, _vp]),
    "fcn_maxpool_fwd_f16": (_i, [_vp, _vp] + [_i] * 12 + [_vp]),
    "fcn_lrn_fwd_f16": (_i, [_vp, _vp, _i, _i, _i, _i, _i, _f, _f, _f, _vp]),
    "fcn_avepool_fwd_f16": (_i, [_vp, _vp] + [_i] * 12 + [_vp]),
    "fcn_deconv_depthwise_fwd_f16": (_i, [_vp, _vp, _vp, _vp] + [_i] * 13 + [_vp]),
    "fcn_eltwise_fwd_f16": (_i, [_vp, _vp, _vp, _sz, _i, _f, _f, _vp]),
    "fcn_softmax_fwd_f16": (_i, [_vp, _vp, _i, _i, _i, _i, _i, _vp]),
    "fcn_copy_channels_f16": (_i, [_vp, _vp, _i, _i, _i, _i, _i, _i, _vp]),
    "fcn_preprocess_bgr8_batch": (_i, [_vp, _i, _i, _i, _vp, _i, _i, _i, _i, _f, _vp, _vp]),
    "fcn_preprocess_bgr8_rois": (_i, [_vp, _i, _i, _vp, _i, _vp, _i, _i, _i, _i, _f, _vp, _vp]),
    "fcn_preprocess_bgr8_f16": (_i, [_vp, _i, _i, _vp, _i, _i, _i, _f, _vp, _vp]),
    "fcn_compose_scene_bgr8": (_i, [_vp, _i, _i, _i, _i, _i, _i, _vp, _i, _i, _vp, _vp, _i, _i, _vp]),
    "fcn_mask_to_label_f32": (_i, [_vp, _i, _i, _vp, _i, _i, _i, _vp]),
    "fcn_compose_scene_view_bgr8": (_i, [_vp, _i, _i, _i, _i, _i, _i, _vp, _i, _i, _vp, _vp, _i, _i, _i, _i, _i, _i, _vp]),
    "fcn_blur_gauss_bgr8": (_i, [_vp, _vp, _vp, _i, _i, _vp, _i, _vp]),
    "fcn_blur_box_bgr8": (_i, [_vp, _vp, _i, _i, _i, _vp]),
    "fcn_blur_median_bgr8": (_i, [_vp, _vp, _i, _i, _i, _vp]),
    "fcn_color_augment_bgr8": (_i, [_vp, _vp, _i, _i, _vp, _vp]),
    "fcn_softmax_fwd_f32": (_i, [_vp, _vp, _i, _i, _i, _i, _vp]),
    "fcn_softmax_loss_workspace_bytes": (_sz, []),
    "fcn_softmax_loss_f32": (_i, [_vp, _vp, _vp, _vp, _i, _i, _i, _i, _i, _i, _i, _i, _f, _vp, _vp]),
    "fcn_deconv_depthwise_bwd_f32": (_i, [_vp, _vp, _vp] + [_i] * 13 + [_vp]),
    "fcn_conv_weights_flip_batch_f32": (_i, [_vp, _vp, _vp, _i, _vp]),
    "fcn_relu_bwd_f32": (_i, [_vp, _vp, _vp, _i, _i, _i, _vp]),
    "fcn_sigmoid_bwd_f32": (_i, [_vp, _vp, _vp, _sz, _i, _vp]),
    "fcn_maxpool_bwd_f32": (_i, [_vp, _vp, _vp] + [_i] * 14 + [_vp]),
    "fcn_maxpool_bwd_mask_f32": (_i, [_vp, _vp, _vp] + [_i] * 14 + [_vp, _i, _i, _vp]),
    "fcn_avepool_bwd_f32": (_i, [_vp, _vp] + [_i] * 14 + [_vp]),
    "fcn_lrn_bwd_f32": (_i, [_vp, _vp, _vp, _vp, _vp, _i, _i, _i, _i, _i, _f, _f, _i, _vp]),
    "fcn_dropout_f32": (_i, [_vp, _vp] + [_i] * 8 + [_f, C.c_uint, C.c_uint, _vp]),
    "fcn_stream_wait_event": (_i, [_vp, _vp]),
    "fcn_comm_unique_id": (_i, [C.c_char_p]),
    "fcn_comm_init": (_i, [C.POINTER(_vp), C.c_char_p, _i, _i]),
    "fcn_comm_allreduce_sum_f32": (_i, [_vp, _vp, _sz, _vp]),
    "fcn_comm_destroy": (_i, [_vp]),
    "fcn_loss_f32": (_i, [_i, _vp, _vp, _vp, _vp, _i, _i, _i, _i, _f, _vp]),
    "fcn_sgd_update_f32": (_i, [_vp, _vp, _vp, _vp, _i, _f, _f, _f, _f, _vp]),
    "fcn_adam_update_f32": (_i, [_vp, _vp, _vp, _vp, _vp, _i, _f, _f, _f, _f, _f, _i, _f, _vp]),
    "fcn_solver_update_f32": (_i, [_i, _vp, _vp, _vp, _vp, _vp, _i, _f, _f, _f, _f, _f, _f, _i, _i, _f, _vp, _vp]),
    "fcn_grad_clip_workspace_bytes": (_sz, []),
    "fcn_grad_clip_f32": (_i, [_vp, _vp, _i, _f, _f, _vp, _vp, _vp, _vp]),
    "fcn_grad_accumulate_f32": (_i, [_vp, _vp, _sz, _i, _vp]),
    "fcn_score_accumulate_f32": (_i, [_vp, _vp, _i, _i, _i, _i, _i, _vp]),
    "fcn_accuracy_workspace_bytes": (_sz, []),
    "fcn_accuracy_f32": (_i, [_vp, _vp, _vp, _vp, _i, _i, _i, _i, _i, _i, _i, _i, _vp, _vp]),
    "fcn_tconv2d_num_configs": (_i, []),
    "fcn_tconv2d_workspace_bytes": (_sz, [C.POINTER(TConvDesc), _i]),
# ... 118 lines not shown
```

### include/fcnhip.h

```cpp
#ifndef FCNHIP_H_
#define FCNHIP_H_

#include <stddef.h>
#include <stdint.h>

#ifdef __cplusplus
extern "C" {
#endif

#define FCN_ABI_VERSION 1

#define FCN_E_ARG       1
#define FCN_E_ALIGN     2
#define FCN_E_UNSUPPORTED 3
#define FCN_E_STATE     4
#define FCN_E_CAPACITY  5

typedef void* fcn_stream_t;
typedef void* fcn_event_t;
typedef void* fcn_graph_t;
typedef void* fcn_comm_t;

int  fcn_abi_version(void);
const char* fcn_last_error_string(void);
int  fcn_device_count(int* count);
int  fcn_init(int device);
int  fcn_device_name(char* h_buf, int len);
int  fcn_device_sync(void);
int  fcn_malloc(void** p, size_t bytes);
int  fcn_free(void* p);
int  fcn_host_malloc(void** h_p, size_t bytes);
int  fcn_host_free(void* h_p);
int  fcn_memset_async(void* p, int value, size_t bytes, fcn_stream_t s);
int  fcn_memcpy_h2d_async(void* dst, const void* h_src, size_t bytes, fcn_stream_t s);
int  fcn_memcpy_d2h_async(void* h_dst, const void* src, size_t bytes, fcn_stream_t s);
int  fcn_memcpy_d2d_async(void* dst, const void* src, size_t bytes, fcn_stream_t s);
int  fcn_stream_create(fcn_stream_t* s);
int  fcn_stream_destroy(fcn_stream_t s);
int  fcn_stream_sync(fcn_stream_t s);
int  fcn_event_create(fcn_event_t* e);
int  fcn_event_destroy(fcn_event_t e);
int  fcn_event_record(fcn_event_t e, fcn_stream_t s);
int  fcn_event_sync(fcn_event_t e);
int  fcn_event_elapsed_ms(fcn_event_t start, fcn_event_t stop, float* h_ms);
int  fcn_stream_wait_event(fcn_stream_t s, fcn_event_t e);
int  fcn_graph_begin(fcn_stream_t s);
int  fcn_graph_end(fcn_stream_t s, fcn_graph_t* g);
int  fcn_graph_launch(fcn_graph_t g, fcn_stream_t s);
int  fcn_graph_destroy(fcn_graph_t g);
#define FCN_REPLICA_STREAMS 4
int  fcn_stream_create_replica(fcn_stream_t* s, int index);
int  fcn_stream_is_prioritized(fcn_stream_t s, int* h_yes);

int  fcn_nchw_to_nhwc_f32(const float* src, float* dst, int N, int C, int H, int W,
                          int dst_cstride, int dst_coffset, float shift, fcn_stream_t s);
int  fcn_nhwc_to_nchw_f32(const float* src, float* dst, int N, int C, int H, int W,
                          int src_cstride, int src_coffset, fcn_stream_t s);
typedef struct fcn_layout_desc {
    const float* src;
    float* dst;
    int32_t N, C, H, W, src_cstride, src_coffset;
} fcn_layout_desc;
int  fcn_nhwc_to_nchw_multi_f32(const fcn_layout_desc* h_descs, int n, fcn_stream_t s);

#define FCN_CONV_RELU      1
#define FCN_CONV_SIGMOID2  2
#define FCN_CONV_ACCUM     4
#define FCN_CONV_MASK     64
#define FCN_CONV_IMAGE_ONES 128
#define FCN_CONV_OUT_F32   8
#define FCN_CONV_OUT_F16  32
#define FCN_CONV_F16      16
typedef struct fcn_conv_desc {
    const float* x;
    const float* w;
    const float* bias;
    float*       y;
    float*       y2;
    int32_t N, H, W, Cin, x_cstride;
    int32_t Cout, kh, kw, pad, stride, OH, OW;
    int32_t y_cstride, y_coffset, y2_cstride, y2_coffset;
    int32_t flags;
    float   in_shift;
} fcn_conv_desc;
int  fcn_conv2d_fwd_f32(const fcn_conv_desc* h_desc, fcn_stream_t s);
typedef struct fcn_conv_group {
    void*   d_probs;
    int32_t n;
    int32_t cfg;
    int32_t total_tiles;
} fcn_conv_group;
size_t fcn_conv2d_group_workspace_bytes(int n);
int  fcn_conv2d_num_configs(void);
int  fcn_conv2d_first_layer_config(void);
typedef struct fcn_conv_tail {
    int32_t n;
    int32_t finalize;
    fcn_conv_desc heads[4];
    float*  scratch;
    void*   arrive;
} fcn_conv_tail;
size_t fcn_conv2d_tail_scratch_bytes(const fcn_conv_tail* t);
size_t fcn_conv2d_tail_arrive_bytes(const fcn_conv_tail* t);
int  fcn_conv2d_group_attach_tail(void* d_workspace, const fcn_conv_tail* t);
int  fcn_conv2d_config_lds_bytes(int cfg);
int  fcn_conv2d_config_waves_k(int cfg);
int  fcn_conv2d_group_prepare(const fcn_conv_desc* h_descs, int n, void* d_workspace, int cfg_request, fcn_conv_group* h_out);
int  fcn_conv2d_fwd_group_f32(const fcn_conv_group* h_group, fcn_stream_t s);
typedef struct fcn_pool_desc {
    const float* x; float* y; int32_t* idx;
    int32_t N, H, W, C, x_cstride, k, stride, pad, OH, OW, y_cstride, y_coffset;
    int32_t f16;
} fcn_pool_desc;
int  fcn_conv2d_group_prepare_fused(const fcn_conv_desc* h_descs, int n, const fcn_pool_desc* h_pools, int npools, void* d_workspace,
                                    int cfg_request, fcn_conv_group* h_out);
int  fcn_conv2d_group_release(void* d_workspace);

int  fcn_maxpool_fwd_f32(const float* x, float* y, int32_t* idx, int N, int H, int W, int C,
                         int x_cstride, int k, int stride, int pad, int OH, int OW,
                         int y_cstride, int y_coffset, fcn_stream_t s);
int  fcn_avepool_fwd_f32(const float* x, float* y, int N, int H, int W, int C, int x_cstride,
                         int k, int stride, int pad, int OH, int OW, int y_cstride, int y_coffset,
                         fcn_stream_t s);
int  fcn_lrn_fwd_f32(const float* x, float* y, float* scale, int pixels, int C, int x_cstride,
                     int y_cstride, int local_size, float alpha, float beta, float k, fcn_stream_t s);
int  fcn_maxpool_lrn5_fwd_f32(const float* x, float* y, int N, int H, int W, int C, int x_cstride, int k, int stride, int pad,
                              int OH, int OW, int y_cstride, int lrn_first, float alpha, float beta, float lrn_k, fcn_stream_t s);
int  fcn_maxpool_lrn5_conv1x1_fwd_f32(const float* x, int N, int H, int W, int C, int x_cstride, int k, int stride, int pad,
                                      int OH, int OW, float alpha, float beta, float lrn_k, const float* w, const float* bias,
                                      int Cout, int relu, float* y, int y_cstride, int y_coffset, fcn_stream_t s);
int  fcn_maxpool_lrn5_conv1x1_fwd_f16(const void* x, int N, int H, int W, int C, int x_cstride, int k, int stride, int pad,
                                      int OH, int OW, float alpha, float beta, float lrn_k, const void* w, const float* bias,
                                      int Cout, int relu, void* y, int y_cstride, int y_coffset, fcn_stream_t s);
int  fcn_relu_fwd_f32(const float* x, float* y, size_t count, float negative_slope, fcn_stream_t s);
int  fcn_sigmoid_fwd_f32(const float* x, float* y, size_t count, fcn_stream_t s);
int  fcn_power_fwd_f32(const float* x, float* y, size_t count, float power, float scale, float shift, fcn_stream_t s);
#define FCN_ELT_PROD 0
#define FCN_ELT_SUM  1
#define FCN_ELT_MAX  2
int  fcn_eltwise_fwd_f32(const float* a, const float* b, float* y, size_t count, int op,
                         float ca, float cb, fcn_stream_t s);
int  fcn_copy_channels_f32(const float* src, float* dst, int pixels, int C, int src_cstride,
                           int src_coffset, int dst_cstride, int dst_coffset, fcn_stream_t s);
int  fcn_softmax_fwd_f32(const float* x, float* y, int pixels, int C, int x_cstride, int y_cstride, fcn_stream_t s);
int  fcn_deconv_depthwise_fwd_f32(const float* x, const float* w, const float* bias, float* y,
                                  int N, int H, int W, int C, int x_cstride, int k, int stride, int pad,
                                  int OH, int OW, int y_cstride, int y_coffset, fcn_stream_t s);

int  fcn_preprocess_bgr8(const uint8_t* frame, int h, int w, float* dst, int H, int W, int dst_cstride,
                         float shift, float* d_minmax, fcn_stream_t s);

int  fcn_nchw_f32_to_nhwc_f16(const float* src, void* dst, int N, int C, int H, int W, int dst_cstride, int dst_coffset, float shift,
                              fcn_stream_t s);
int  fcn_nhwc_f16_to_nchw_f32(const void* src, float* dst, int N, int C, int H, int W, int src_cstride, int src_coffset, fcn_stream_t s);
int  fcn_maxpool_fwd_f16(const void* x, void* y, int N, int H, int W, int C, int x_cstride, int k, int stride, int pad, int OH, int OW,
                         int y_cstride, int y_coffset, fcn_stream_t s);
int  fcn_lrn_fwd_f16(const void* x, void* y, int pixels, int C, int x_cstride, int y_cstride, int local_size, float alpha, float beta,
                     float k, fcn_stream_t s);
int  fcn_maxpool_lrn5_fwd_f16(const void* x, void* y, int N, int H, int W, int C, int x_cstride, int k, int stride, int pad,
                              int OH, int OW, int y_cstride, int lrn_first, float alpha, float beta, float lrn_k, fcn_stream_t s);
int  fcn_avepool_fwd_f16(const void* x, void* y, int N, int H, int W, int C, int x_cstride, int k, int stride, int pad, int OH, int OW,
                         int y_cstride, int y_coffset, fcn_stream_t s);
int  fcn_deconv_depthwise_fwd_f16(const void* x, const float* w, const float* bias, void* y, int N, int H, int W, int C, int x_cstride,
                                  int k, int stride, int pad, int OH, int OW, int y_cstride, int y_coffset, int out_f32, fcn_stream_t s);
int  fcn_eltwise_fwd_f16(const void* a, const void* b, void* y, size_t count, int op, float ca, float cb, fcn_stream_t s);
int  fcn_softmax_fwd_f16(const void* x, void* y, int pixels, int C, int x_cstride, int y_cstride, int out_f32, fcn_stream_t s);
int  fcn_copy_channels_f16(const void* src, void* dst, int pixels, int C, int src_cstride, int src_coffset, int dst_cstride,
                           int dst_coffset, fcn_stream_t s);
int  fcn_preprocess_bgr8_rois(const uint8_t* frame, int h, int w, const int32_t* h_rois, int n, void* dst, int dst_f16, int H, int W,
                              int dst_cstride, float shift, float* d_minmax, fcn_stream_t s);
int  fcn_preprocess_bgr8_batch(const uint8_t* frames, int n, int h, int w, void* dst, int dst_f16, int H, int W, int dst_cstride,
                               float shift, float* d_minmax, fcn_stream_t s);
int  fcn_preprocess_bgr8_f16(const uint8_t* frame, int h, int w, void* dst, int H, int W, int dst_cstride, float shift, float* d_minmax,
                             fcn_stream_t s);

typedef struct fcn_scene_obj {
    const uint8_t* img;
    const uint8_t* mask;
    int32_t src_h, src_w;
    int32_t flip;
    int32_t roi_x, roi_y, roi_w, roi_h;
    int32_t out_w, out_h;
    int32_t cx, cy;
    int32_t label1;
} fcn_scene_obj;
int  fcn_compose_scene_bgr8(const uint8_t* bg, int bg_h, int bg_w, int crop_x, int crop_y, int crop_w, int crop_h,
                            const fcn_scene_obj* d_objs, int nobj, int final_flip, uint8_t* out_img, uint8_t* out_mask,
                            int H, int W, fcn_stream_t s);
int  fcn_compose_scene_view_bgr8(const uint8_t* bg, int bg_h, int bg_w, int crop_x, int crop_y, int crop_w, int crop_h,
                                 const fcn_scene_obj* d_objs, int nobj, int final_flip, uint8_t* out_img, uint8_t* out_mask,
                                 int H, int W, int view_x, int view_y, int view_w, int view_h, fcn_stream_t s);
// ... 328 lines not shown
```

Before: 4558 frames/s.

## Read planar input directly in first conv, band uploads, and mirror outputs to NCHW

The first 7x7 conv kernel gains a planar variant that reads the uploaded NCHW image directly, applying the mean shift, and skips the separate NCHW-to-NHWC conversion pass. An optional banded upload pipelines host-to-device copies of row bands on a copy stream with first-layer compute on each band. The 1x1 head kernel can also write NCHW mirror outputs directly, so the final layout conversion before download is dropped. Together these remove per-frame layout kernels and overlap input transfer with compute, at the cost of more complex graph capture and extra events and streams.

```diff
diff --git a/fcn_object_detector_amd/csrc/common.h b/fcn_object_detector_amd/csrc/common.h
--- a/fcn_object_detector_amd/csrc/common.h
+++ b/fcn_object_detector_amd/csrc/common.h
@@ -34,6 +34,7 @@
     } while (0)
 
 const float* zero_page_for_current_device(int* rc);
+int first7_geometry(const fcn_conv_group* g, int* H, int* W, int* OH);
 
 inline int cdiv(long long a, long long b) { return (int)((a + b - 1) / b); }
 
diff --git a/fcn_object_detector_amd/csrc/conv_fwd.hip b/fcn_object_detector_amd/csrc/conv_fwd.hip
--- a/fcn_object_detector_amd/csrc/conv_fwd.hip
+++ b/fcn_object_detector_amd/csrc/conv_fwd.hip
@@ -1002,41 +1002,66 @@
 constexpr int kD7Threads = 256;
 static_assert(kD7LdsBytes <= 80 * 1024, "first-layer kernel: two workgroups per CU");
 
-__global__ __launch_bounds__(kD7Threads) void conv_first7_kernel(const ConvP p) {
+template <bool PLANAR>
+__device__ __forceinline__ void conv_first7_body(const ConvP& p, const float* __restrict__ planar, const float shift, const int oy_begin, const int oy_end,
+                                                 float* smem) {
 #if defined(__HIP_DEVICE_COMPILE__)
-    __shared__ __attribute__((aligned(16))) float smem[kD7LdsBytes / 4];
     const int tid = threadIdx.x, lane = tid & 63, wave = __builtin_amdgcn_readfirstlane(tid >> 6);
     FCN_STAMP(0);
-    const int tiles_x = (p.OW + kD7Tw - 1) / kD7Tw, tiles_y = (p.OH + kD7Th - 1) / kD7Th;
+    const int tiles_x = (p.OW + kD7Tw - 1) / kD7Tw, tiles_y = (oy_end - oy_begin + kD7Th - 1) / kD7Th;
     int t = blockIdx.x;
     const int tx = t % tiles_x;
     t /= tiles_x;
     const int ty = t % tiles_y, n = t / tiles_y;
-    const int oy0 = ty * kD7Th, ox0 = tx * kD7Tw;
+    const int oy0 = oy_begin + ty * kD7Th, ox0 = tx * kD7Tw;
     const int iy0 = 2 * oy0 - 3, ix0 = 2 * ox0 - 3;
     const v4f zero4 = {0.f, 0.f, 0.f, 0.f};
     constexpr int PI = (kD7Ph * kD7Pw + kD7Threads - 1) / kD7Threads, WI = (64 * 49 + kD7Threads - 1) / kD7Threads;
-    v4f px[PI], wv[WI];
-    const float* xn = p.x + (size_t)n * p.H * p.W * 4;
-#pragma unroll
-    for (int i = 0; i < PI; ++i) {
-        const int s = tid + kD7Threads * i;
-        const int pr = s / kD7Pw, pc = s - pr * kD7Pw;
-        const int iy = iy0 + pr, ix = ix0 + pc;
-        const bool ok = s < kD7Ph * kD7Pw && (unsigned)iy < (unsigned)p.H && (unsigned)ix < (unsigned)p.W;
-        px[i] = ok ? *reinterpret_cast<const v4f*>(xn + ((size_t)iy * p.W + ix) * 4) : zero4;
+    constexpr int QT = 3 * kD7Pw;
+    v4f px[PLANAR ? 1 : PI], wv[WI];
+    float pq[PLANAR ? kD7Ph : 1];
+    const int qc = tid / kD7Pw, qpc = tid - qc * kD7Pw;
+    if constexpr (PLANAR) {
+        const int iy_end = min(p.H, 2 * oy_end + 2);
+        const int ix = ix0 + qpc;
+        const bool col_ok = tid < QT && (unsigned)ix < (unsigned)p.W;
+        const float* src = planar + (size_t)(col_ok ? qc : 0) * p.H * p.W + (col_ok ? ix : 0);
+#pragma unroll
+        for (int pr = 0; pr < kD7Ph; ++pr) {
+            const int iy = iy0 + pr;
+            const bool ok = col_ok && iy >= 0 && iy < iy_end;
+            pq[pr] = ok ? src[(size_t)iy * p.W] + shift : 0.f;
+        }
+    } else {
+        const float* xn = p.x + (size_t)n * p.H * p.W * 4;
+#pragma unroll
+        for (int i = 0; i < PI; ++i) {
+            const int s = tid + kD7Threads * i;
+            const int pr = s / kD7Pw, pc = s - pr * kD7Pw;
+            const int iy = iy0 + pr, ix = ix0 + pc;
+            const bool ok = s < kD7Ph * kD7Pw && (unsigned)iy < (unsigned)p.H && (unsigned)ix < (unsigned)p.W;
+            px[i] = ok ? *reinterpret_cast<const v4f*>(xn + ((size_t)iy * p.W + ix) * 4) : zero4;
+        }
     }
 #pragma unroll
     for (int i = 0; i < WI; ++i) {
         const int tp = tid + kD7Threads * i;
         wv[i] = tp < p.Cout * 49 ? *reinterpret_cast<const v4f*>(p.w + (size_t)tp * 4) : zero4;
     }
-#pragma unroll
-    for (int i = 0; i < PI; ++i) {
-        const int s = tid + kD7Threads * i;
-        if (s < kD7Ph * kD7Pw) {
-            float* d = smem + s * 3;
-            d[0] = px[i][0]; d[1] = px[i][1]; d[2] = px[i][2];
+    if constexpr (PLANAR) {
+        if (tid < QT) {
+            float* d = smem + qpc * 3 + qc;
+#pragma unroll
+            for (int pr = 0; pr < kD7Ph; ++pr) d[pr * kD7RowF] = pq[pr];
+        }
+    } else {
+#pragma unroll
+        for (int i = 0; i < PI; ++i) {
+            const int s = tid + kD7Threads * i;
+            if (s < kD7Ph * kD7Pw) {
+                float* d = smem + s * 3;
+                d[0] = px[i][0]; d[1] = px[i][1]; d[2] = px[i][2];
+            }
         }
     }
 #pragma unroll
@@ -1109,7 +1134,7 @@
             if (do_relu)
 #pragma unroll
                 for (int e = 0; e < 4; ++e) v[e] = fmaxf(v[e], 0.f);
-            if (oy < p.OH && ox0 + ox < p.OW && c4 < p.Cout) *reinterpret_cast<v4f*>(yrow + (size_t)ox * p.y_cstride) = v;
+            if (oy < oy_end && ox0 + ox < p.OW && c4 < p.Cout) *reinterpret_cast<v4f*>(yrow + (size_t)ox * p.y_cstride) = v;
         }
     }
 #ifdef FCN_CONV_STAMPS
@@ -1118,6 +1143,17 @@
     FCN_STAMP(6);
 #endif
 #endif
+}
+
+__global__ __launch_bounds__(kD7Threads) void conv_first7_kernel(const ConvP p) {
+    __shared__ __attribute__((aligned(16))) float smem[kD7LdsBytes / 4];
+    conv_first7_body<false>(p, nullptr, 0.f, 0, p.OH, smem);
+}
+
+__global__ __launch_bounds__(kD7Threads) void conv_first7_planar_kernel(const ConvP p, const float* __restrict__ planar, const float shift,
+                                                                        const int oy_begin, const int oy_end) {
+    __shared__ __attribute__((aligned(16))) float smem[kD7LdsBytes / 4];
+    conv_first7_body<true>(p, planar, shift, oy_begin, oy_end, smem);
 }
 
 constexpr int kH7PatchSlots = (kD7Ph * kD7Pw + 63) / 64 * 64;
@@ -1470,10 +1506,12 @@
     const float* bias;
     float* y;
     float* y2;
-    int K, x_cstride, y_cstride, y_coffset, y2_cstride, y2_coffset, nout, flags;
+    float* yn;
+    float* yn2;
+    int K, x_cstride, y_cstride, y_coffset, y2_cstride, y2_coffset, nout, flags, cout;
 };
 struct DotArgs {
-    int M, nslices;
+    int M, nslices, HW;
     DotSlice s[kDotMaxSlices];
 };
 
@@ -1535,7 +1573,14 @@
                 if (sl.bias) v += sl.bias[o];
                 if (sl.flags & FCN_CONV_RELU) v = fmaxf(v, 0.f);
                 sl.y[(size_t)m * sl.y_cstride + sl.y_coffset + o] = v;
-                if (sl.flags & FCN_CONV_SIGMOID2) sl.y2[(size_t)m * sl.y2_cstride + sl.y2_coffset + o] = 1.f / (1.f + expf(-v));
+                const int img = m / a.HW;
+                const size_t mn = ((size_t)img * sl.cout + o) * a.HW + (m - img * a.HW);
+                if (sl.yn) sl.yn[mn] = v;
+                if (sl.flags & FCN_CONV_SIGMOID2) {
+                    const float sg = 1.f / (1.f + expf(-v));
+                    sl.y2[(size_t)m * sl.y2_cstride + sl.y2_coffset + o] = sg;
+                    if (sl.yn2) sl.yn2[mn] = sg;
+                }
             }
         }
         asm volatile("s_waitcnt lgkmcnt(0)" ::: "memory");
@@ -1853,7 +1898,9 @@
 }
 
 struct HostTail { bool on; int finalize; int n; fcn_conv_desc heads[kTailMaxSlices]; float* scratch; unsigned* arrive; TailP t; };
-struct HostGroup { int n; ConvP ps[16]; int npool; PoolP pools[kMaxPool]; HostTail tail; };
+constexpr int kMaxMirrors = 4;
+struct HostMirror { const float* nhwc; int coffset; float* nchw; };
+struct HostGroup { int n; ConvP ps[16]; int npool; PoolP pools[kMaxPool]; HostTail tail; int nmirror; HostMirror mirrors[kMaxMirrors]; };
 std::unordered_map<const void*, HostTail> g_tails;
 std::mutex g_groups_mu;
 std::unordered_map<const void*, HostGroup> g_groups;
@@ -2011,6 +2058,7 @@
         hg.npool = npools;
         for (int i = 0; i < kMaxPool; ++i) hg.pools[i] = pools[i];
         hg.tail = tail;
+        hg.nmirror = 0;
     }
     h_out->d_probs = d_workspace;
     h_out->n = n;
@@ -2083,6 +2131,43 @@
     return 0;
 }
 
+int fcn_conv2d_group_mirror_nchw(const fcn_conv_group* g, const float* nhwc, int coffset, float* nchw) {
+    FCN_REQUIRE(g && g->d_probs && nhwc && nchw, FCN_E_ARG, "fcn_conv2d_group_mirror_nchw: null");
+    FCN_REQUIRE(g->cfg == kDot1x1Cfg, FCN_E_UNSUPPORTED, "fcn_conv2d_group_mirror_nchw: only the lane-split 1x1 kernel (configuration %d) writes mirrors", kDot1x1Cfg);
+    std::lock_guard<std::mutex> lock(g_groups_mu);
+    auto it = g_groups.find(g->d_probs);
+    FCN_REQUIRE(it != g_groups.end() && it->second.n == g->n, FCN_E_STATE, "fcn_conv2d_group_mirror_nchw: group was not prepared by this library instance");
+    HostGroup& hg = it->second;
+    bool found = false;
+    for (int i = 0; i < hg.n; ++i) {
+        const ConvP& q = hg.ps[i];
+        found = found || (q.y == nhwc && q.y_coffset == coffset) || ((q.flags & FCN_CONV_SIGMOID2) && q.y2 == nhwc && q.y2_coffset == coffset);
+    }
+    FCN_REQUIRE(found, FCN_E_ARG, "fcn_conv2d_group_mirror_nchw: no problem of the group writes that blob");
+    FCN_REQUIRE(hg.nmirror < kMaxMirrors, FCN_E_UNSUPPORTED, "fcn_conv2d_group_mirror_nchw: at most %d mirrors per group", kMaxMirrors);
+    hg.mirrors[hg.nmirror++] = HostMirror{nhwc, coffset, nchw};
+    return 0;
+}
+
+int fcn_conv2d_first_planar_f32(const fcn_conv_group* g, const float* planar, float shift, int oy_begin, int oy_end, fcn_stream_t s) {
+    FCN_REQUIRE(g && g->d_probs && planar, FCN_E_ARG, "fcn_conv2d_first_planar_f32: null");
+    FCN_REQUIRE(g->cfg == kFirst7Cfg && g->n == 1, FCN_E_UNSUPPORTED, "fcn_conv2d_first_planar_f32: a group prepared for the first-layer kernel (configuration %d)", kFirst7Cfg);
+    ConvP p;
+    {
+        std::lock_guard<std::mutex> lock(g_groups_mu);
+        auto it = g_groups.find(g->d_probs);
+        FCN_REQUIRE(it != g_groups.end() && it->second.n == 1 && it->second.npool == 0, FCN_E_STATE, "fcn_conv2d_first_planar_f32: group was not prepared by this library instance");
+        p = it->second.ps[0];
+    }
+    FCN_REQUIRE(first7_ok(p) && p.N == 1, FCN_E_UNSUPPORTED, "fcn_conv2d_first_planar_f32: one float32 image (batch 1), float32 output");
+    FCN_REQUIRE(((uintptr_t)planar & 3) == 0 && 3ll * p.H * p.W < (1ll << 31), FCN_E_ARG, "fcn_conv2d_first_planar_f32: planar image misaligned or too large");
+    FCN_REQUIRE(oy_begin >= 0 && oy_begin < oy_end && oy_end <= p.OH, FCN_E_ARG, "fcn_conv2d_first_planar_f32: rows [%d, %d) of %d", oy_begin, oy_end, p.OH);
+    const int tiles = cdiv(p.OW, kD7Tw) * cdiv(oy_end - oy_begin, kD7Th);
+    hipLaunchKernelGGL(conv_first7_planar_kernel, dim3(tiles), dim3(kD7Threads), 0, as_stream(s), p, planar, shift, oy_begin, oy_end);
+    FCN_LAUNCH_CHECK("conv_first7_planar");
+    return 0;
+}
+
 int fcn_conv2d_fwd_group_f32(const fcn_conv_group* g, fcn_stream_t s) {
     FCN_REQUIRE(g && g->d_probs && g->n > 0 && g->total_tiles > 0, FCN_E_ARG, "fcn_conv2d_fwd_group_f32: unprepared group");
     FCN_REQUIRE(g->cfg >= 0 && g->cfg < num_cfgs(), FCN_E_ARG, "fcn_conv2d_fwd_group_f32: bad cfg %d", g->cfg);
@@ -2097,6 +2182,7 @@
         FCN_REQUIRE(hg.npool == 0 && dot1x1_ok(hg.ps, hg.n), FCN_E_STATE, "fcn_conv2d_fwd_group_f32: group was not prepared for the lane-split 1x1 kernel");
         DotArgs da = {};
         da.M = hg.ps[0].M;
+        da.HW = hg.ps[0].OH * hg.ps[0].OW;
         for (int i = 0; i < hg.n; ++i)
             for (int n0 = 0; n0 < hg.ps[i].Cout; n0 += kDotOut) {
                 const ConvP& q = hg.ps[i];
@@ -2106,6 +2192,12 @@
                 d.y2_cstride = q.y2_cstride; d.y2_coffset = q.y2_coffset + n0;
                 d.nout = q.Cout - n0 < kDotOut ? q.Cout - n0 : kDotOut;
                 d.flags = q.flags;
+                d.cout = q.Cout;
+                for (int k = 0; k < hg.nmirror; ++k) {
+                    const HostMirror& mr = hg.mirrors[k];
+                    if (mr.nhwc == q.y && mr.coffset == q.y_coffset) d.yn = mr.nchw + (size_t)n0 * da.HW;
+                    if ((q.flags & FCN_CONV_SIGMOID2) && mr.nhwc == q.y2 && mr.coffset == q.y2_coffset) d.yn2 = mr.nchw + (size_t)n0 * da.HW;
+                }
             }
         hipLaunchKernelGGL(conv_dot1x1_kernel, dim3(g->total_tiles), dim3(64 * kDotMaxSlices), 0, as_stream(s), da);
         FCN_LAUNCH_CHECK("conv_dot1x1");
@@ -2187,3 +2279,14 @@
 }
 
 }
+
+int fcn::first7_geometry(const fcn_conv_group* g, int* H, int* W, int* OH) {
+    FCN_REQUIRE(g && g->d_probs && g->cfg == kFirst7Cfg && g->n == 1, FCN_E_UNSUPPORTED, "frame plan: a group prepared for the first-layer kernel (configuration %d)", kFirst7Cfg);
+    std::lock_guard<std::mutex> lock(g_groups_mu);
+    auto it = g_groups.find(g->d_probs);
+    FCN_REQUIRE(it != g_groups.end() && it->second.n == 1, FCN_E_STATE, "frame plan: group was not prepared by this library instance");
+    const ConvP& p = it->second.ps[0];
+    FCN_REQUIRE(first7_ok(p) && p.N == 1, FCN_E_UNSUPPORTED, "frame plan: one float32 image (batch 1), float32 output");
+    *H = p.H; *W = p.W; *OH = p.OH;
+    return 0;
+}
diff --git a/fcn_object_detector_amd/csrc/runtime.hip b/fcn_object_detector_amd/csrc/runtime.hip
--- a/fcn_object_detector_amd/csrc/runtime.hip
+++ b/fcn_object_detector_amd/csrc/runtime.hip
@@ -212,4 +212,84 @@
     return 0;
 }
 
-}
+struct FramePlan {
+    fcn_conv_group first;
+    int H, W, OH;
+    int bands;
+    int oy[FCN_FRAME_MAX_BANDS + 1];
+    int iy[FCN_FRAME_MAX_BANDS + 1];
+    hipStream_t copy;
+    hipEvent_t ready[FCN_FRAME_MAX_BANDS];
+    hipEvent_t idle;
+};
+
+int fcn_frame_plan_create(const fcn_conv_group* first, int bands, fcn_frame_plan_t* h_plan) {
+    FCN_REQUIRE(first && h_plan, FCN_E_ARG, "fcn_frame_plan_create: null");
+    FCN_REQUIRE(bands >= 1 && bands <= FCN_FRAME_MAX_BANDS, FCN_E_ARG, "fcn_frame_plan_create: 1..%d bands", FCN_FRAME_MAX_BANDS);
+    FramePlan* fp = new FramePlan();
+    fp->first = *first;
+    int rc = first7_geometry(first, &fp->H, &fp->W, &fp->OH);
+    if (rc) {
+        delete fp;
+        return rc;
+    }
+    fp->oy[0] = fp->iy[0] = 0;
+    int nb = 0;
+    for (int i = 1; i <= bands; ++i) {
+        int end = i == bands ? fp->OH : (int)((long long)fp->OH * i / bands + 7) / 8 * 8;
+        if (end > fp->OH) end = fp->OH;
+        if (end <= fp->oy[nb]) continue;
+        ++nb;
+        fp->oy[nb] = end;
+        fp->iy[nb] = end == fp->OH ? fp->H : (2 * end + 4 < fp->H ? 2 * end + 4 : fp->H);
+    }
+    fp->bands = nb;
+    if (nb > 1) {
+        hipError_t e = hipStreamCreateWithFlags(&fp->copy, hipStreamNonBlocking);
+        for (int i = 0; e == hipSuccess && i < nb; ++i) e = hipEventCreateWithFlags(&fp->ready[i], hipEventDisableTiming);
+        if (e == hipSuccess) e = hipEventCreateWithFlags(&fp->idle, hipEventDisableTiming);
+        if (e != hipSuccess) {
+            fcn_frame_plan_destroy(fp);
+            return set_err(-(int)e, "fcn_frame_plan_create: %s", hipGetErrorString(e));
+        }
+    }
+    *h_plan = fp;
+    return 0;
+}
+
+int fcn_frame_plan_destroy(fcn_frame_plan_t plan) {
+    FramePlan* fp = (FramePlan*)plan;
+    if (!fp) return 0;
+    for (int i = 0; i < FCN_FRAME_MAX_BANDS; ++i)
+        if (fp->ready[i]) (void)hipEventDestroy(fp->ready[i]);
+    if (fp->idle) (void)hipEventDestroy(fp->idle);
+    if (fp->copy) (void)hipStreamDestroy(fp->copy);
+    delete fp;
+    return 0;
+}
+
+int fcn_frame_plan_bands(fcn_frame_plan_t plan) { return plan ? ((FramePlan*)plan)->bands : -1; }
+
+int fcn_frame_upload_banded(fcn_frame_plan_t plan, const float* h_frame, float* d_planar, float shift, fcn_stream_t s) {
+    FramePlan* fp = (FramePlan*)plan;
+    FCN_REQUIRE(fp && h_frame && d_planar, FCN_E_ARG, "fcn_frame_upload_banded: null");
+    const size_t plane = (size_t)fp->H * fp->W;
+    if (fp->bands == 1) {
+        FCN_HIP(hipMemcpyAsync(d_planar, h_frame, 3 * plane * sizeof(float), hipMemcpyHostToDevice, as_stream(s)));
+        return fcn_conv2d_first_planar_f32(&fp->first, d_planar, shift, 0, fp->OH, s);
+    }
+    FCN_HIP(hipEventRecord(fp->idle, as_stream(s)));
+    FCN_HIP(hipStreamWaitEvent(fp->copy, fp->idle, 0));
+    for (int b = 0; b < fp->bands; ++b) {
+        const size_t off = (size_t)fp->iy[b] * fp->W, count = (size_t)(fp->iy[b + 1] - fp->iy[b]) * fp->W;
+        for (int c = 0; c < 3 && count; ++c)
+            FCN_HIP(hipMemcpyAsync(d_planar + c * plane + off, h_frame + c * plane + off, count * sizeof(float), hipMemcpyHostToDevice, fp->copy));
+        FCN_HIP(hipEventRecord(fp->ready[b], fp->copy));
+        FCN_HIP(hipStreamWaitEvent(as_stream(s), fp->ready[b], 0));
+        int rc = fcn_conv2d_first_planar_f32(&fp->first, d_planar, shift, fp->oy[b], fp->oy[b + 1], s);
+        if (rc) return rc;
+    }
+    return 0;
+}
+
+}
diff --git a/fcn_object_detector_amd/engine.py b/fcn_object_detector_amd/engine.py
--- a/fcn_object_detector_amd/engine.py
+++ b/fcn_object_detector_amd/engine.py
@@ -307,7 +307,8 @@
                  params: Optional[Dict[str, List[np.ndarray]]] = None, device: int = 0,
                  fuse: bool = True, group_convs: bool = True, autotune: bool = True, dtype: str = "f32",
                  tune_from: Optional["Engine"] = None, tune_max_lds_kb: Optional[int] = None,
-                 share_params: Optional["Engine"] = None, score_outputs: bool = False, replica: Optional[int] = None):
+                 share_params: Optional["Engine"] = None, score_outputs: bool = False, replica: Optional[int] = None,
+                 frame_bands: Optional[int] = None):
         if dtype not in ("f32", "f16"):
             raise ValueError("dtype must be 'f32' or 'f16'")
         if share_params is not None and (dtype != "f32" or share_params.f16):
@@ -344,6 +345,7 @@
         self.ops: List[Op] = []
         self.graph_io: Optional[int] = None
         self.graph_core: Optional[int] = None
+        self.graph_frame: Optional[int] = None
         self._staging: Dict[str, DeviceBuffer] = {}
         self._keep: List[object] = []
         self._conv_layer_meta: Dict[str, dict] = {}
@@ -353,6 +355,7 @@
         self._bn_ws_bytes = 0
         self._bn_ws: Optional[DeviceBuffer] = None
         self._lazy_blob_ops: Dict[str, List[Op]] = {}
+        self._conv_launches: List[Tuple[List[ConvTask], L.ConvGroup, Op]] = []
         self.loss_blobs: Dict[str, float] = {}
         self.device_fed: set = set()
         self.dropout_seed = 0
@@ -365,6 +368,7 @@
         self._plan_buffers()
         self._alloc_params(params)
         self._build_ops()
+        self._plan_frame_path(int(os.environ.get("FCN_FRAME_BANDS", "0")) if frame_bands is None else int(frame_bands))
         self.tuner.release()
 
     @property
@@ -1050,6 +1054,8 @@
         if tailed:
             label = "%s {%s %s}" % (label, "tail:" if tail["desc"].finalize else "partial sums of", "+".join(ht.layer.name for ht in tail["heads"]))
         self.ops.append(Op(kind, label, lambda st, g=grp: L.check(lib.fcn_conv2d_fwd_group_f32(C.byref(g), st)), flops, byts))
+        if getattr(self, "_conv_launches", None) is not None:
+            self._conv_launches.append((chunk, grp, self.ops[-1]))
 
     def _emit_convs(self, items: List[ConvTask], pools: List[OpTask], tail: Optional[dict]) -> None:
         for base in range(0, len(items), 16):
@@ -1577,6 +1583,78 @@
             xb.ptr, wdev, bdev, yb.buf.ptr, g.n, g.h, g.w, c, xb.cstride, k, g.s, g.pad, g.oh, g.ow, yb.cstride, yb.coffset, *out_f32, st)),
             2.0 * yb.pixels * c * (k / g.s) ** 2, float(xb.esize * xb.pixels + yb.esize * yb.pixels) * c)]
 
+    def _plan_frame_path(self, bands: int) -> None:
+        self._planar: Optional[dict] = None
+        self._mirrored = False
+        self._frame_plan: Optional[int] = None
+        self._frame_bands = max(int(bands), 0)
+        self._inputs_stale: set = set()
+        if self.f16 or self.spec.phase != "TEST" or self.score_outputs or os.environ.get("FCN_FRAME_PATH", "1") == "0":
+            return
+        lib = L.load()
+        first7 = int(lib.fcn_conv2d_first_layer_config())
+        special = set(self.detections) | set(self.permutes) | set(self.rpn_views) | set(self.spec.prior_blobs) | set(self.roi_counts)
+        outs = [self.blobs[nm] for nm in self.outputs]
+        if outs and os.environ.get("FCN_FRAME_HEADS", "1") != "0" and \
+                all(b.nchw is not None and b.esize == 4 and not b.lazy_shift and b.name not in special for b in outs):
+            for chunk, grp, _ in self._conv_launches:
+                if grp.cfg != first7 + 1:
+                    continue
+                descs = [t.desc for t in chunk]
+
+                def written(b: Blob) -> bool:
+                    return any((d.y == b.buf.ptr and d.y_coffset == b.coffset and d.Cout == b.channels and d.y_cstride == b.cstride) or
+                               ((d.flags & L.CONV_SIGMOID2) and d.y2 == b.buf.ptr and d.y2_coffset == b.coffset and d.Cout == b.channels
+                                and d.y2_cstride == b.cstride) for d in descs)
+                if not all(written(b) for b in outs) or len(outs) > 4:
+                    continue
+                counts = [int(np.prod(b.shape)) for b in outs]
+                self._out_stage = DeviceBuffer(4 * sum(counts), zero=True)
+                self._out_pinned = PinnedArray((sum(counts),))
+                off = 0
+                for b, cnt in zip(outs, counts):
+                    self._staging[b.name] = DevView(self._out_stage.ptr + 4 * off, 4 * cnt)
+                    b.host = self._out_pinned.array[off:off + cnt].reshape(b.shape)
+                    L.call("fcn_conv2d_group_mirror_nchw", C.byref(grp), b.buf.ptr, b.coffset, self._staging[b.name].ptr)
+                    off += cnt
+                self._mirrored = True
+                break
+        for nm in self.inputs if self._frame_bands >= 1 else ():
+            b = self.blobs[nm]
+            if b.nchw is None or b.esize != 4 or b.nchw[:2] != (1, 3) or b.cstride != 4 or b.coffset != 0 or not self.ops:
+                continue
+            hit = [(chunk, grp, op) for chunk, grp, op in self._conv_launches if any(t.desc.x == b.ptr for t in chunk)]
+            if len(hit) != 1 or len(hit[0][0]) != 1 or hit[0][1].cfg != first7 or hit[0][2] is not self.ops[0]:
+                continue
+            chunk, grp, op = hit[0]
+            readers = [l.name for l in self.spec.layers if any(bt in self.blobs and self.blobs[bt].buf is b.buf for bt in l.bottoms)
+                       and not (l.type == "Power" and l.tops and l.tops[0] in self.shift)]
+            if readers != [chunk[0].layer.name]:
+                continue
+            self._planar = dict(name=nm, group=grp, op=op, oh=int(chunk[0].desc.OH))
+            break
+
+    def _planar_now(self) -> bool:
+        return self._planar is not None and self._planar["name"] not in self.device_fed
+
+    def _first_planar(self, stream: Optional[int]) -> None:
+        nm, grp = self._planar["name"], self._planar["group"]
+        L.check(L.load().fcn_conv2d_first_planar_f32(C.byref(grp), self._stage(nm).ptr, self.blobs[nm].upload_shift, 0, self._planar["oh"], stream))
+
+    def _frame_upload(self, stream: Optional[int]) -> None:
+        nm = self._planar["name"]
+        if self._frame_plan is None:
+            fp = C.c_void_p()
+            L.call("fcn_frame_plan_create", C.byref(self._planar["group"]), self._frame_bands, C.byref(fp))
+            self._frame_plan = int(fp.value)
+        host = self.host_array(nm)
+        L.check(L.load().fcn_frame_upload_banded(self._frame_plan, host.ctypes.data, self._stage(nm).ptr, self.blobs[nm].upload_shift, stream))
+
+    def _materialize_inputs(self, stream: Optional[int]) -> None:
+        for nm in sorted(self._inputs_stale):
+            self._upload_convert(nm, stream)
+        self._inputs_stale.clear()
+
     def _stage(self, name: str) -> DeviceBuffer:
         st = self._staging.get(name)
         if st is None:
@@ -1600,6 +1678,7 @@
 
     def _upload_convert(self, name: str, stream: Optional[int]) -> None:
         b = self.blobs[name]
+        self._inputs_stale.discard(name)
         if b.nchw is None:
             return
         lib = L.load()
@@ -1677,6 +1756,7 @@
             b = self.blobs[name]
             host = self.host_array(name)
             if not b.host_valid:
+                self._materialize_inputs(self.stream)
                 for op in self._lazy_blob_ops.get(name, ()):
                     op.run(self.stream)
                 self._enqueue_download(name, self.stream)
@@ -1795,7 +1875,7 @@
         for op in self.ops:
             op.run(stream)
 
-    def _capture(self, with_io: bool, download: bool = True) -> int:
+    def _capture(self, with_io: bool, download: bool = True, frame: bool = False) -> int:
         if with_io:
             for nm in list(self.inputs) + list(self.outputs):
                 self.host_array(nm)
@@ -1814,14 +1894,28 @@
                 self._download_copy(nm, self.stream)
             L.call("fcn_stream_sync", self.stream)
             self._warm_io = True
+        planar = frame and self._planar_now()
+        if planar and not getattr(self, "_warm_frame", False):
+            if self._frame_bands > 1:
+                self._frame_upload(self.stream)
+            else:
+                self._first_planar(self.stream)
+            L.call("fcn_stream_sync", self.stream)
+            self._warm_frame = True
+        if frame:
+            self._frame_planar = planar
         L.call("fcn_graph_begin", self.stream)
         try:
             if with_io:
                 for nm in self.inputs:
-                    if nm not in self.device_fed:
+                    if nm not in self.device_fed and not (planar and nm == self._planar["name"]):
                         self._upload_convert(nm, self.stream)
-            self.run_ops(self.stream)
-            if with_io and download:
+            for op in self.ops:
+                if not (planar and op is self._planar["op"]):
+                    op.run(self.stream)
+                elif self._frame_bands == 1:
+                    self._first_planar(self.stream)
+            if with_io and download and not (frame and self._mirrored):
                 self._download_convert_all(self.stream)
         finally:
             g = C.c_void_p()
@@ -1837,6 +1931,32 @@
         L.call("fcn_graph_launch", self.graph_io, self.stream)
         for nm in self.outputs:
             self._download_copy(nm, self.stream)
+        self._download_counts(self.stream)
+
+    def _launch_frame(self) -> None:
+        if self._planar is None and not self._mirrored:
+            return self._launch_io()
+        if self.graph_frame is not None and self._frame_planar != self._planar_now():
+            L.call("fcn_graph_destroy", self.graph_frame)
+            self.graph_frame = None
+        if self.graph_frame is None:
+            self.graph_frame = self._capture(with_io=True, frame=True)
+        for nm in self.inputs:
+            if nm in self.device_fed:
+                continue
+            planar = self._frame_planar and nm == self._planar["name"]
+            if planar and self._frame_bands > 1:
+                self._frame_upload(self.stream)
+            else:
+                self._upload_copy(nm, self.stream)
+            if planar:
+                self._inputs_stale.add(nm)
+        L.call("fcn_graph_launch", self.graph_frame, self.stream)
+        if self._mirrored:
+            L.check(L.load().fcn_memcpy_d2h_async(self._out_pinned.ptr, self._out_stage.ptr, self._out_stage.nbytes, self.stream))
+        else:
+            for nm in self.outputs:
+                self._download_copy(nm, self.stream)
         self._download_counts(self.stream)
 
     def forward(self, use_graph: bool = True) -> Dict[str, np.ndarray]:
@@ -1878,7 +1998,7 @@
             for nm in list(self.inputs) + list(self.outputs):
                 self.host_array(nm)
             if graphs_enabled():
-                self._launch_io()
+                self._launch_frame()
             else:
                 for nm in self.inputs:
                     if nm not in self.device_fed:
@@ -1913,6 +2033,7 @@
 
     def forward_enqueue(self) -> None:
         with self.lock:
+            self._materialize_inputs(self.stream)
             if graphs_enabled():
                 if self.graph_core is None:
                     self.graph_core = self._capture(with_io=False)
@@ -1928,6 +2049,7 @@
         use_graph = use_graph and graphs_enabled()
         with self.lock:
             L.call("fcn_init", self.device)
+            self._materialize_inputs(self.stream)
             if use_graph and self.graph_core is None:
                 self.graph_core = self._capture(with_io=False)
             e0, e1 = C.c_void_p(), C.c_void_p()
@@ -1954,6 +2076,7 @@
     def time_ops(self, reps: int = 20, ops: Optional[Sequence["Op"]] = None) -> List[Tuple[str, str, float, float, float]]:
         out = []
         with self.lock:
+            self._materialize_inputs(self.stream)
             e0, e1 = C.c_void_p(), C.c_void_p()
             L.call("fcn_event_create", C.byref(e0))
             L.call("fcn_event_create", C.byref(e1))
@@ -1974,6 +2097,7 @@
     def time_ops_in_sequence(self, reps: int = 10) -> List[Tuple[str, str, float, float, float]]:
         out = []
         with self.lock:
+            self._materialize_inputs(self.stream)
             e0, e1 = C.c_void_p(), C.c_void_p()
             L.call("fcn_event_create", C.byref(e0))
             L.call("fcn_event_create", C.byref(e1))
@@ -2007,12 +2131,15 @@
     def close(self) -> None:
         with self.lock:
             lib = L.load()
-            for g in (self.graph_io, self.graph_core, self.graph_score):
+            for g in (self.graph_io, self.graph_core, self.graph_score, getattr(self, "graph_frame", None)):
                 if g:
                     lib.fcn_graph_destroy(g)
-            self.graph_io = self.graph_core = self.graph_score = None
+            self.graph_io = self.graph_core = self.graph_score = self.graph_frame = None
             if self.stream:
                 lib.fcn_stream_sync(self.stream)
+                if getattr(self, "_frame_plan", None):
+                    lib.fcn_frame_plan_destroy(self._frame_plan)
+                    self._frame_plan = None
                 lib.fcn_stream_destroy(self.stream)
                 self.stream = 0
             for ws in getattr(self, "_group_workspaces", []):
@@ -2118,6 +2245,8 @@
         for e in engines:
             if e.graph_core is None:
                 e.forward_resident(1)
+            with e.lock:
+                e._materialize_inputs(e.stream)
             L.call("fcn_stream_sync", e.stream)
         no_graph = not graphs_enabled()
         t0 = time.perf_counter()
diff --git a/fcn_object_detector_amd/lib.py b/fcn_object_detector_amd/lib.py
--- a/fcn_object_detector_amd/lib.py
+++ b/fcn_object_detector_amd/lib.py
@@ -212,6 +212,10 @@
     "fcn_graph_destroy": (_i, [_vp]),
     "fcn_stream_create_replica": (_i, [C.POINTER(_vp), _i]),
     "fcn_stream_is_prioritized": (_i, [_vp, C.POINTER(_i)]),
+    "fcn_frame_plan_create": (_i, [C.POINTER(ConvGroup), _i, C.POINTER(_vp)]),
+    "fcn_frame_plan_destroy": (_i, [_vp]),
+    "fcn_frame_plan_bands": (_i, [_vp]),
+    "fcn_frame_upload_banded": (_i, [_vp, _vp, _vp, _f, _vp]),
     "fcn_nchw_to_nhwc_f32": (_i, [_vp, _vp, _i, _i, _i, _i, _i, _i, _f, _vp]),
     "fcn_nhwc_to_nchw_f32": (_i, [_vp, _vp, _i, _i, _i, _i, _i, _i, _vp]),
     "fcn_nhwc_to_nchw_multi_f32": (_i, [C.POINTER(LayoutDesc), _i, _vp]),
@@ -224,6 +228,8 @@
     "fcn_conv2d_group_prepare": (_i, [C.POINTER(ConvDesc), _i, _vp, _i, C.POINTER(ConvGroup)]),
     "fcn_conv2d_group_prepare_fused": (_i, [C.POINTER(ConvDesc), _i, C.POINTER(PoolDesc), _i, _vp, _i, C.POINTER(ConvGroup)]),
     "fcn_conv2d_fwd_group_f32": (_i, [C.POINTER(ConvGroup), _vp]),
+    "fcn_conv2d_first_planar_f32": (_i, [C.POINTER(ConvGroup), _vp, _f, _i, _i, _vp]),
+    "fcn_conv2d_group_mirror_nchw": (_i, [C.POINTER(ConvGroup), _vp, _i, _vp]),
     "fcn_conv2d_group_release": (_i, [_vp]),
     "fcn_conv2d_tail_scratch_bytes": (C.c_size_t, [C.POINTER(ConvTail)]),
     "fcn_conv2d_tail_arrive_bytes": (C.c_size_t, [C.POINTER(ConvTail)]),
diff --git a/include/fcnhip.h b/include/fcnhip.h
--- a/include/fcnhip.h
+++ b/include/fcnhip.h
@@ -51,6 +51,13 @@
 #define FCN_REPLICA_STREAMS 4
 int  fcn_stream_create_replica(fcn_stream_t* s, int index);
 int  fcn_stream_is_prioritized(fcn_stream_t s, int* h_yes);
+#define FCN_FRAME_MAX_BANDS 8
+typedef void* fcn_frame_plan_t;
+struct fcn_conv_group;
+int  fcn_frame_plan_create(const struct fcn_conv_group* first, int bands, fcn_frame_plan_t* h_plan);
+int  fcn_frame_plan_destroy(fcn_frame_plan_t plan);
+int  fcn_frame_plan_bands(fcn_frame_plan_t plan);
+int  fcn_frame_upload_banded(fcn_frame_plan_t plan, const float* h_frame, float* d_planar, float shift, fcn_stream_t s);
 
 int  fcn_nchw_to_nhwc_f32(const float* src, float* dst, int N, int C, int H, int W,
                           int dst_cstride, int dst_coffset, float shift, fcn_stream_t s);
@@ -107,6 +114,8 @@
 int  fcn_conv2d_config_waves_k(int cfg);
 int  fcn_conv2d_group_prepare(const fcn_conv_desc* h_descs, int n, void* d_workspace, int cfg_request, fcn_conv_group* h_out);
 int  fcn_conv2d_fwd_group_f32(const fcn_conv_group* h_group, fcn_stream_t s);
+int  fcn_conv2d_first_planar_f32(const fcn_conv_group* h_group, const float* planar, float shift, int oy_begin, int oy_end, fcn_stream_t s);
+int  fcn_conv2d_group_mirror_nchw(const fcn_conv_group* h_group, const float* nhwc, int coffset, float* nchw);
 typedef struct fcn_pool_desc {
     const float* x; float* y; int32_t* idx;
     int32_t N, H, W, C, x_cstride, k, stride, pad, OH, OW, y_cstride, y_coffset;
```

After: 4528 frames/s. About the same (-0.6%).
